# EarthyScience/EasyHybrid.jl

Measured on AMD Instinct MI355X. Metric: training samples/sec, higher is better.
Workload: dtype f32; 1 GPU; RbQ10 hybrid, MLP [2,16,16,1] tanh -> rb (sigmoid-scaled), Q10 global, MSE + Adam(0.01), batch=65536 per GPU, fp32 (BASELINE.json configs[1]); global_batch=65536, resident_batches_per_gpu=64, parallelism=dp1, ranks_seen=1, launcher=none, gradient_exchange=none (one GPU)

## Files before the change

### easyhybrid.jl_amd/csrc/eh_api.hip

```cpp
#include <hip/hip_runtime.h>
#include <chrono>

#include <algorithm>
#include <cfloat>
#include <atomic>
#include <cmath>
#include <cstdarg>
#include <cstdio>
#include <cstdlib>
#include <cstring>
#include <memory>
#include <mutex>
#include <string>
#include <thread>
#include <vector>

#include "eh_internal.hpp"
#include "eh_kernels.hpp"
#include "eh_chain.hpp"
#include "eh_lbfgs.hpp"
#include "eh_wide.hpp"
#include "eh_lform.hpp"
#include "eh_seq.hpp"

// ... 277 lines not shown
    const EhNet& net = h->net;
    EhStepArgs v = *a;
    v.fz.gacc = nullptr;
    v.count = std::min<long long>(a->count, 8192);
    v.bn_update = 0; v.stamps = nullptr; v.slab = h->slab; v.n_acc = h->n_acc;
    v.yhat = nullptr; v.pout = nullptr;
    if (v.count <= 0) return true;
    const int grid = grid_for(h, v.count);
    const size_t nb = (size_t)h->n_acc * sizeof(float);
    float* dev = nullptr;
    if (hipMalloc(&dev, 2 * nb) != hipSuccess) { (void)hipGetLastError(); return true; }
    std::vector<float> host(2 * (size_t)h->n_acc);
    float* sc = h->sc;
    bool launched = true;
    for (int k = 0; k < 2 && launched; ++k) {
        hipError_t e = k == 0 ? h->arch->var[h->variant].launch(EH_MODE_TRAIN, h->act, KFAST(h), grid, h->stream, &net, &v)
                              : eh_jit_launch(&je->k, EH_MODE_TRAIN, grid, h->stream, &net, &v);
        if (e != hipSuccess) { (void)hipGetLastError(); launched = false; break; }
        hipLaunchKernelGGL((eh_reduce_kernel<false, 16>), dim3((h->n_acc + 15) / 16), dim3(256), 0, h->stream, h->slab, grid, h->n_acc, net.n_theta, net.T, 0,
                           dev + (size_t)k * h->n_acc, TH(h), MM(h), VV(h), sc, sc, h->opt, (float*)nullptr, h->img, net.loss, (const float*)nullptr, (const float*)nullptr, 0u);
        if (hipGetLastError() != hipSuccess) { launched = false; break; }
    }
    bool ok = true;
    std::string why;
    if (launched && hipMemcpyAsync(host.data(), dev, 2 * nb, hipMemcpyDeviceToHost, h->stream) == hipSuccess && hipStreamSynchronize(h->stream) == hipSuccess) {
        const float* A = host.data(); const float* B = A + h->n_acc;
        if (getenv("EH_DEBUG_JIT_SKEW")) host[(size_t)h->n_acc + net.n_theta] *= 1.01f;
        double gmax = 0.0, dmax = 0.0;
        for (int i = 0; i < net.n_theta; ++i) { gmax = std::max(gmax, (double)fabsf(A[i])); dmax = std::max(dmax, (double)fabsf(A[i] - B[i])); }
        const double sa = A[net.n_theta], sb = B[net.n_theta];
        bool counts = true;
        for (int t = 0; t < net.T; ++t) counts = counts && A[net.n_theta + 1 + t] == B[net.n_theta + 1 + t];
        const bool loss_ok = (std::isnan(sa) && std::isnan(sb)) || fabs(sa - sb) <= 1e-5 * fabs(sa) + 1e-30;
        if (!(dmax <= 1e-5 * gmax + 1e-30) || !loss_ok || !counts || !std::isfinite(gmax)) {
            ok = false;
            char b[320];
            snprintf(b, sizeof b, "the kernel compiled at run time disagrees with the one built ahead of time on %lld samples of this model's data "
                     "(gradient: max |difference| %.3g against a largest entry of %.3g; loss sum %.9g vs %.9g; valid counts %s): the handle keeps the kernels built ahead of time",
                     v.count, dmax, gmax, sb, sa, counts ? "equal" : "DIFFERENT");
            why = b;
        }
    } else (void)hipGetLastError();
    (void)hipFree(dev);
    if (!ok) { je->state.store(-1); h->jit_failed = true; h->jit_log = why; }
    return ok;
}

static void eh_agg_factors(eh_handle* h) {
    int tdata = 0;
    for (int t = 0; t < h->net.T; ++t) tdata += ((h->roles >> (2 * t)) & 3u) == 0u ? 1 : 0;
    h->img.agg_a = h->agg ? 1.0f / ((float)std::max(1, tdata) * (float)(1 + h->n_extra)) : 1.0f;
    h->img.l2s = h->agg ? 1.0f / (float)(1 + h->n_extra) : 1.0f;
}

static const EhSpecKernel* spec_lookup(const eh_handle* h) {
    static const EhSpecKernel* const list[] = {
#define EH_SPEC_ITEM(k) eh_spec_##k(),
        EH_SPEC_LIST(EH_SPEC_ITEM)
#undef EH_SPEC_ITEM
    };
    static std::mutex mu;
    static uint64_t prepared[sizeof list / sizeof list[0]] = {};
    if (!h->aot_spec || h->lform || h->act == EH_ACT_PER_NET || h->drop_on) return nullptr;
    const EhArchInfo* A = h->arch;
    const EhVariant& V = A->var[h->variant];
    const int kf = KFAST(h);
    for (size_t i = 0; i < sizeof list / sizeof list[0]; ++i) {
        const EhSpecKernel* k = list[i];
        if (k->wide != (A->wide != 0) || k->bf16 != V.bf16 || k->nbi != A->nbi || k->nbh != A->nbh || k->nl != A->nl || k->nt != V.nt || k->nw != V.nw ||
            k->act != h->act || k->fast != kf || (k->so != 0) != (V.so != 0) || memcmp(&k->net, &h->net, sizeof(EhNet)) != 0) continue;
        {
            std::lock_guard<std::mutex> lk(mu);
            const uint64_t bit = 1ull << (h->device & 63);
            if (!(prepared[i] & bit)) {
                if (hipSetDevice(h->device) != hipSuccess || k->prepare() != hipSuccess) { (void)hipGetLastError(); return nullptr; }
                prepared[i] |= bit;
            }
        }
        return k;
    }
    return nullptr;
}

static hipError_t step_launch(eh_handle* h, int mode, int grid, const EhStepArgs* a) {
    if (mode == EH_MODE_TRAIN_ORD) {
        if (const EhSpecKernel* sk = spec_lookup(h)) {
            const hipError_t e = sk->launch(mode, grid, h->stream, &h->net, a);
            if (e == hipSuccess) h->spec_used = sk; else (void)hipGetLastError();
            return e;
        }
        if (jit_wanted(h, EH_MODE_TRAIN)) {
            eh_handle_s::JitEntry* je = jit_entry(h);
            if (je) return (je->verified && je->k.fn[EH_MODE_TRAIN_ORD]) ? eh_jit_launch(&je->k, mode, grid, h->stream, &h->net, a) : hipErrorNotSupported;
        }
        return h->arch->var[h->variant].launch(mode, h->act, KFAST(h), grid, h->stream, &h->net, a);
    }
    if (mode == EH_MODE_TRAIN_MULTI) {
        if (const EhSpecKernel* sk = spec_lookup(h)) {
            if (sk->launch(mode, grid, h->stream, &h->net, a) == hipSuccess) { h->spec_used = sk; return hipSuccess; }
            (void)hipGetLastError();
        } else if (jit_wanted(h, EH_MODE_TRAIN)) {
            eh_handle_s::JitEntry* je = jit_entry(h);
            if (je && je->verified && je->k.fn[EH_MODE_TRAIN_MULTI]) {
                if (eh_jit_launch(&je->k, mode, grid, h->stream, &h->net, a) == hipSuccess) return hipSuccess;
                (void)hipGetLastError();
            }
        }
        return h->arch->var[h->variant].launch(mode, h->act, KFAST(h), grid, h->stream, &h->net, a);
    }
    if (const EhSpecKernel* sk = spec_lookup(h)) {
        const hipError_t e = sk->launch(mode, grid, h->stream, &h->net, a);
        if (e == hipSuccess) { h->spec_used = sk; return e; }
        (void)hipGetLastError();
    }
    if (jit_wanted(h, mode)) {
        eh_handle_s::JitEntry* je = jit_entry(h);
        if (je && !je->verified && mode != EH_MODE_EVAL && !h->capturing && je->spec && h->net.mech != EH_MECH_PROGRAM && h->net.loss != EH_LOSS_PROGRAM &&
            h->act != EH_ACT_PER_NET && !h->drop_on && !getenv("EH_JIT_NO_VERIFY")) {
            bool has_lprog = false;
            for (int t = 0; t < h->net.T; ++t) has_lprog = has_lprog || ((h->net.loss_t >> (4 * t)) & 15u) == (unsigned)EH_LOSS_PROGRAM;
            if (has_lprog || jit_verify(h, je, a)) je->verified = true; else je = nullptr;
        }
        if (je) {
            const hipError_t e = eh_jit_launch(&je->k, mode, grid, h->stream, &h->net, a);
            if (e == hipSuccess) return e;
            (void)hipGetLastError();
            je->state.store(-1); h->jit_failed = true;
            h->jit_log = std::string("launch of the run-time compiled kernel failed: ") + hipGetErrorString(e);
        }
        if ((h->net.loss == EH_LOSS_PROGRAM || h->drop_on) && mode != EH_MODE_EVAL) return hipErrorNotSupported;
    }
    if (h->act == EH_ACT_PER_NET) return hipErrorNotSupported;
    return h->arch->var[h->variant].launch(mode, h->act, KFAST(h), grid, h->stream, &h->net, a);
}

extern "C" {

int32_t eh_version(void) { return EH_ABI_VERSION; }

const char* eh_last_error(const eh_handle* h) { return h ? h->err.c_str() : g_create_err.c_str(); }

static std::mutex g_stage_mu;
static float* g_stage[2] = {nullptr, nullptr};
static size_t g_stage_bytes = 0;
static int copy_out(eh_handle* h, float* dst, const float* src_dev, size_t n);
static void lbfgs_release(eh_handle* h);
static int copy_in(eh_handle* h, float* dst_dev, const float* src, size_t n);
static std::mutex g_stream_pool_mu;
static std::vector<std::pair<int, hipStream_t>> g_stream_pool;
static hipStream_t stream_pool_take(int device) {
    std::lock_guard<std::mutex> lk(g_stream_pool_mu);
    for (size_t i = 0; i < g_stream_pool.size(); ++i)
        if (g_stream_pool[i].first == device) { hipStream_t s = g_stream_pool[i].second; g_stream_pool.erase(g_stream_pool.begin() + (long)i); return s; }
    return nullptr;
}
static void stream_pool_give(int device, hipStream_t s) {
    {
        std::lock_guard<std::mutex> lk(g_stream_pool_mu);
        int kept = 0;
        for (auto& e : g_stream_pool) kept += e.first == device;
        if (kept < 8 && !getenv("EH_NO_STREAM_POOL")) { g_stream_pool.emplace_back(device, s); return; }
    }
    (void)hipStreamDestroy(s);
}

static int seq_desc_check(const eh_model_desc* d) {
    if (d->activation != EH_ACT_PER_NET) return 0;
    const int na = std::min(d->n_nets > 0 ? d->n_nets : d->n_hidden, (int)EH_MAX_NETS);
    int n_lstm = 0, at = -1;
    for (int l = 0; l < na; ++l)
        if (d->net_activation[l] == EH_LAYER_LSTM) { if (at < 0) at = l; ++n_lstm; }
    if (!n_lstm) return 0;
    if (d->n_nets > 0) return fail(nullptr, EH_EUNSUPPORTED, "eh_create: no kernel for a MultiNN sequence model (EH_LAYER_LSTM with n_nets = %d)", d->n_nets);
    if (at == 0) return fail(nullptr, EH_EINVAL, "eh_create: EH_LAYER_LSTM at hidden layer 0: the LSTM layer takes the Dense layer in front of it");
    if (n_lstm > 1) return fail(nullptr, EH_EINVAL, "eh_create: %d EH_LAYER_LSTM layers (one, at hidden layer 1: stacked Recurrence layers are not built)", n_lstm);
    if (d->n_hidden != 3 || at != 1 || d->hidden[2] != d->hidden[1])
        return fail(nullptr, EH_EUNSUPPORTED, "eh_create: no kernel for an LSTM layer at hidden layer %d of %d (built: n_hidden = 3, hidden = [I, H, H], the LSTM at layer 1)", at, d->n_hidden);
    if (d->hidden[0] < 1 || d->hidden[1] < 1) return fail(nullptr, EH_EINVAL, "eh_create: hidden = [%d, %d, ..]", d->hidden[0], d->hidden[1]);
    if (d->hidden[0] > 32 || d->hidden[1] > 32) return fail(nullptr, EH_EUNSUPPORTED, "eh_create: no kernel for LSTM widths I = %d, H = %d (built: up to 32 each)", d->hidden[0], d->hidden[1]);
    if (d->n_predictors > 32) return fail(nullptr, EH_EUNSUPPORTED, "eh_create: no kernel for a sequence model with P = %d predictors (built: up to 32)", d->n_predictors);
    if (d->input_batchnorm) return fail(nullptr, EH_EUNSUPPORTED, "eh_create: no kernel for input BatchNorm on a sequence model (3-D input)");
    if (d->n_targets > 1) return fail(nullptr, EH_EUNSUPPORTED, "eh_create: no kernel for a sequence model with %d targets (built: one)", d->n_targets);
    return 1;
}

int32_t eh_create(const eh_model_desc* d, eh_handle** out) {
    if (!d || !out) return fail(nullptr, EH_EINVAL, "eh_create: null argument");
    *out = nullptr;
    if (d->struct_size != (int32_t)sizeof(eh_model_desc)) return fail(nullptr, EH_EINVAL, "eh_create: struct_size %d != %zu", d->struct_size, sizeof(eh_model_desc));
    MechInfo mi;
    if (!mech_info(d->mech, &mi, d)) return fail(nullptr, EH_EUNSUPPORTED, "eh_create: unknown mechanistic model id %d (no silent fallback)", d->mech);
    const int seqk = (d->activation == EH_ACT_PER_NET && d->n_hidden >= 0 && d->n_hidden <= EH_MAX_HIDDEN && d->n_nets >= 0 && d->n_nets <= EH_MAX_NETS) ? seq_desc_check(d) : 0;
    if (seqk < 0) return seqk;
    const bool seq = seqk == 1;
    if (d->mech == EH_MECH_PROGRAM) {
        if (d->n_params < 1 || d->n_params > EH_MAX_PARAMS) return fail(nullptr, EH_EINVAL, "eh_create: a program takes 1..%d parameters, descriptor has %d", EH_MAX_PARAMS, d->n_params);
        if (d->prog_len < 1 || d->prog_len > EH_MAX_PROG) return fail(nullptr, EH_EUNSUPPORTED, "eh_create: program of %d instructions (1..%d)", d->prog_len, EH_MAX_PROG);
        if (d->prog_n_const < 0 || d->prog_n_const > EH_MAX_PROG_CONST) return fail(nullptr, EH_EUNSUPPORTED, "eh_create: program with %d constants (0..%d)", d->prog_n_const, EH_MAX_PROG_CONST);
        if (d->prog_n_forc < 0 || d->prog_n_forc > EH_MAX_FORC) return fail(nullptr, EH_EINVAL, "eh_create: program with %d forcings (0..%d)", d->prog_n_forc, EH_MAX_FORC);
        if (d->prog_n_out < 1 || d->prog_n_out > EH_MAX_PROG_OUT) return fail(nullptr, EH_EUNSUPPORTED, "eh_create: program with %d outputs (1..%d)", d->prog_n_out, EH_MAX_PROG_OUT);
        auto slot_ok = [&](unsigned sl, int upto) {
            if (sl < EH_PROG_SLOT_FORC) return (int)sl < d->n_params;
            if (sl < EH_PROG_SLOT_CONST) return (int)sl - EH_PROG_SLOT_FORC < d->prog_n_forc;
            if (sl < EH_PROG_SLOT_INSTR) return (int)sl - EH_PROG_SLOT_CONST < d->prog_n_const;
            return (int)sl - EH_PROG_SLOT_INSTR < upto;
        };
        for (int i = 0; i < d->prog_len; ++i) {
            const unsigned w = d->prog_code[i], op = w & 255u;
            if (op >= EH_OP_COUNT) return fail(nullptr, EH_EUNSUPPORTED, "eh_create: program instruction %d has unknown opcode %u", i, op);
            const int nop = (op == EH_OP_SELECT) ? 3 : (op == EH_OP_NEG || op == EH_OP_EXP || op == EH_OP_LOG || op == EH_OP_SQRT || op == EH_OP_TANH ||
                                                        op == EH_OP_SIGMOID || op == EH_OP_ABS || op == EH_OP_SIN || op == EH_OP_COS) ? 1 : 2;
            const unsigned sl[3] = {(w >> 8) & 255u, (w >> 16) & 255u, w >> 24};
            for (int k = 0; k < 3; ++k) {
                if (k < nop ? !slot_ok(sl[k], i) : sl[k] != 0u)
                    return fail(nullptr, EH_EINVAL, "eh_create: program instruction %d, operand %d names slot %u (undefined at that point, or a non-zero unused operand)", i, k, sl[k]);
// ... 276 lines not shown
    }
    tick("pset / bn / gacc");
    h->slab_rows = lform ? (int)EH_LFORM_ROWS : h->max_blocks;
    HIPCHK_C(hipMalloc(&h->slab, (std::max((size_t)h->slab_rows * std::max(h->n_acc, EH_EVAL_STATS * n.T), (size_t)1 << 20) + 16) * sizeof(float)));
    HIPCHK_C(hipMalloc(&h->gradbuf, (size_t)h->n_acc * sizeof(float)));
    HIPCHK_C(hipMalloc(&h->mombuf, EH_MAX_TARG * EH_EVAL_STATS * sizeof(float)));
    HIPCHK_C(hipMemset(h->mombuf, 0, EH_MAX_TARG * EH_EVAL_STATS * sizeof(float)));
    HIPCHK_C(hipMalloc(&h->tcount, 3 * EH_MAX_TARG * sizeof(float)));
    HIPCHK_C(hipMemset(h->tcount, 0, 3 * EH_MAX_TARG * sizeof(float)));
    HIPCHK_C(hipMalloc(&h->inv_n, EH_TT * EH_MAX_TARG * sizeof(float)));
    HIPCHK_C(hipMemset(h->inv_n, 0, EH_TT * EH_MAX_TARG * sizeof(float)));
    HIPCHK_C(hipMemset(h->gradbuf, 0, (size_t)h->n_acc * sizeof(float)));
    tick("slab + small buffers");
    if (seq) {
        std::vector<unsigned char> wf((size_t)n.n_theta, 0);
        const int* o = h->seq_off;
        std::fill(wf.begin() + o[EH_SEQ_WIN], wf.begin() + o[EH_SEQ_BIN], (unsigned char)1);
        std::fill(wf.begin() + o[EH_SEQ_WHD], wf.begin() + o[EH_SEQ_BHD], (unsigned char)1);
        std::fill(wf.begin() + o[EH_SEQ_WOUT], wf.begin() + o[EH_SEQ_BOUT], (unsigned char)1);
        HIPCHK_C(hipMalloc(&h->wflag, wf.size()));
        HIPCHK_C(hipMemcpy(h->wflag, wf.data(), wf.size(), hipMemcpyHostToDevice));
    }
    else if (!lform) { if (int rc = build_maps(h, true)) { g_create_err = h->err; eh_destroy(h); return rc; } }
    else {
        std::vector<unsigned char> wf((size_t)n.n_theta, 0);
        for (int k = 0; k < h->l_nnets; ++k)
            for (int l = 0; l < h->l_net[k].nl; ++l) std::fill(wf.begin() + h->l_net[k].woff[l], wf.begin() + h->l_net[k].boff[l], (unsigned char)1);
        HIPCHK_C(hipMalloc(&h->wflag, wf.size()));
        HIPCHK_C(hipMemcpy(h->wflag, wf.data(), wf.size(), hipMemcpyHostToDevice));
    }
    tick("maps");
    {
        std::vector<float> img0((size_t)arch->img_floats, 0.0f);
        for (int j = 0; j < d->n_params; ++j) {
            if (d->param_kind[j] == EH_PAR_FIXED) img0[arch->phi_off + EH_IMG_PHI + j] = d->param_default[j];
            img0[arch->phi_off + EH_IMG_LO + j] = d->param_lower[j];
            img0[arch->phi_off + EH_IMG_SC + j] = d->param_upper[j] - d->param_lower[j];
        }
        for (int p = 0; p < 32; ++p) { img0[arch->phi_off + EH_IMG_BNM + p] = 0.0f; img0[arch->phi_off + EH_IMG_BNR + p] = d->input_batchnorm ? 1.0f / std::sqrt(1.0f + EH_BN_EPS) : 1.0f; }
        for (int k = 0; k < (lform ? 0 : n_nets); ++k)
            for (int l = net_d[k]; l < nl; ++l)
                for (int i = 0; i < net_w[k][l]; ++i)
                    img0[arch->wh_off + (size_t)(l - 1) * arch->hp * arch->sh + (size_t)(h->net_r0[k][l] + i) * arch->sh + h->net_r0[k][l - 1] + i] = 1.0f;
        auto put_int = [&](int slot, int v) { memcpy(&img0[arch->phi_off + slot], &v, sizeof(int)); };
        if (!lform && !seq) {
            for (int l = 0; l <= d->n_hidden; ++l) { put_int(EH_IMG_WOFF + l, lw_off[l]); put_int(EH_IMG_BOFF + l, lb_off[l]); }
            for (int l = 0; l < d->n_hidden; ++l) put_int(EH_IMG_WIDTH + l, tot_w[l]);
        }
        for (int j = 0; j < d->n_params; ++j)
            if (d->param_kind[j] == EH_PAR_GLOBAL) put_int(EH_IMG_GPAR + d->param_index[j], j);
        HIPCHK_C(hipMalloc(&h->image, img0.size() * sizeof(float)));
        HIPCHK_C(hipMemcpy(h->image, img0.data(), img0.size() * sizeof(float), hipMemcpyHostToDevice));
        EhImg& im = h->img;
        im.image = h->image; im.imap = h->imap; im.g_off = n.g_off; im.phi_off = arch->phi_off;
        im.l2c = 0.0f; im.l2w = nullptr; im.n_theta = n.n_theta; im.b_off = arch->b_off; im.wflag = h->wflag;
        im.agg_a = 1.0f; im.l2s = 1.0f;
        HIPCHK_C(hipMalloc(&h->l2val, sizeof(float)));
        HIPCHK_C(hipMemset(h->l2val, 0, sizeof(float)));
        {
            int nw = 0;
            if (seq) nw = (h->seq_off[EH_SEQ_BIN] - h->seq_off[EH_SEQ_WIN]) + (h->seq_off[EH_SEQ_BHD] - h->seq_off[EH_SEQ_WHD]) + (h->seq_off[EH_SEQ_BOUT] - h->seq_off[EH_SEQ_WOUT]);
            else if (lform) { for (int k = 0; k < h->l_nnets; ++k) for (int l = 0; l < h->l_net[k].nl; ++l) nw += h->l_net[k].in[l] * h->l_net[k].out[l]; }
            else for (const EhEntry& e : enumerate_entries(h)) nw += e.col >= 0 ? 1 : 0;
            h->n_weights = nw;
        }
        for (int j = 0; j < d->n_params; ++j)
            if (d->param_kind[j] == EH_PAR_GLOBAL) {
                const int g = d->param_index[j];
                im.glob_par[g] = j; im.glo[g] = d->param_lower[j]; im.ghi[g] = d->param_upper[j];
            }
        tick("image");
        hipLaunchKernelGGL(eh_image_kernel, dim3((unsigned)((nt + 255) / 256)), dim3(256), 0, h->stream, TH(h), (int)nt, h->img);
        HIPCHK_C(hipGetLastError());
        tick("image kernel launch");
        HIPCHK_C(hipStreamSynchronize(h->stream));
        tick("synchronize");
    }
#undef HIPCHK_C
    if (h->act == EH_ACT_PER_NET && !h->lform && !h->seq && !jit_entry(h)) {
        const std::string log = h->jit_log;
        eh_destroy(h);
        return fail(nullptr, EH_EUNSUPPORTED, "eh_create: per-net activations need the run-time compiled kernel, which failed to build: %.600s", log.c_str());
    }
    *out = h;
    return EH_OK;
}

int32_t eh_destroy(eh_handle* h) {
    if (!h) return EH_OK;
    (void)hipSetDevice(h->device);
    if (h->own_stream) (void)hipStreamSynchronize(h->own_stream);
    for (auto e : h->ev) (void)hipEventDestroy(e);
    for (auto& g : h->graphs) (void)hipGraphExecDestroy(g.exec);
    for (auto& e : h->jit) { if (e->worker.joinable()) e->worker.join(); eh_jit_release(&e->k); }
    eh_comm_release(h);
    (void)hipSetDevice(h->device);
    (void)hipFree(h->pset); (void)hipFree(h->opt_tab);
    (void)hipFree(h->gacc); (void)hipFree(h->ord); if (h->ord_err) (void)hipHostFree(h->ord_err); (void)hipFree(h->bn_part); (void)hipFree(h->bn_run); (void)hipFree(h->bn_shift); (void)hipFree(h->bn_stat); (void)hipFree(h->tcount); (void)hipFree(h->mombuf); (void)hipFree(h->slab); (void)hipFree(h->gradbuf); (void)hipFree(h->inv_n);
    (void)hipFree(h->prog); (void)hipFree(h->l2val); (void)hipFree(h->l2w); (void)hipFree(h->loss_hist); (void)hipFree(h->perm); (void)hipFree(h->out_buf); (void)hipFree(h->idx_buf);
    eval_host_release(h);
    lbfgs_release(h);
    (void)hipFree(h->mech_ws); (void)hipFree(h->l_ws); (void)hipFree(h->l_split); (void)hipFree(h->l_dk); (void)hipFree(h->l_lprog); (void)hipFree(h->wflag);
    (void)hipFree(h->stamps); (void)hipFree(h->image); (void)hipFree(h->imap); (void)hipFree(h->rmap);
    (void)hipFree(h->split[0].recs); (void)hipFree(h->split[1].recs); (void)hipFree(h->split[0].starts); (void)hipFree(h->split[1].starts); (void)hipFree(h->seq_ws); (void)hipFree(h->chain_part);
    if (h->own_stream) stream_pool_give(h->device, h->own_stream);
    delete h;
    return EH_OK;
}

int32_t eh_n_theta(const eh_handle* h, int64_t* n) {
    if (!h || !n) return EH_EINVAL;
    *n = h->net.n_theta;
    return EH_OK;
}

int32_t eh_set_stream(eh_handle* h, void* s) {
    if (!h) return EH_EINVAL;
    h->stream = s ? (hipStream_t)s : h->own_stream;
    return EH_OK;
}

int32_t eh_synchronize(eh_handle* h) {
    if (!h) return EH_EINVAL;
    HIPCHK(h, hipSetDevice(h->device));
    FLUSH(h);
    HIPCHK(h, hipStreamSynchronize(h->stream));
    if (h->p2p_on) {
        unsigned c[3] = {0, 0, 0};
        HIPCHK(h, hipMemcpy(c, h->p2p_ctr, sizeof c, hipMemcpyDeviceToHost));
        if (c[1]) return fail(h, EH_EHIP, "eh_synchronize: a cross-GPU exchange ran into its 2 s deadline (a rank is missing or out of step); results are invalid");
    }
    if (h->ord_err && *(volatile unsigned*)h->ord_err)
        return fail(h, EH_EHIP, "eh_synchronize: an ordered step's row of sums did not arrive within its 2 s deadline; results are invalid");
    return EH_OK;
}

static int set_loss_program(eh_handle* h, int target, const uint32_t* code, int32_t n_instr, const float* consts, int32_t n_const, int32_t out_slot, const char* who) {
    if (!h || !code || (n_const > 0 && !consts)) return EH_EINVAL;
    if (h->seq) return fail(h, EH_EUNSUPPORTED, "%s: recorded losses are not built for sequence models", who);
    if (n_instr < 1 || n_instr > EH_MAX_PROG) return fail(h, EH_EUNSUPPORTED, "%s: %d instructions (1..%d)", who, n_instr, EH_MAX_PROG);
    if (n_const < 0 || n_const > EH_MAX_PROG_CONST) return fail(h, EH_EUNSUPPORTED, "%s: %d constants (0..%d)", who, n_const, EH_MAX_PROG_CONST);
    auto slot_ok = [&](unsigned sl, int upto) {
        if (sl < EH_PROG_SLOT_CONST) return sl < 2u;
        if (sl < EH_PROG_SLOT_INSTR) return (int)sl - EH_PROG_SLOT_CONST < n_const;
        return (int)sl - EH_PROG_SLOT_INSTR < upto;
    };
    for (int i = 0; i < n_instr; ++i) {
        const unsigned w = code[i], op = w & 255u;
        if (op >= EH_OP_COUNT) return fail(h, EH_EUNSUPPORTED, "%s: instruction %d has unknown opcode %u", who, i, op);
        const int nop = (op == EH_OP_SELECT) ? 3 : (op == EH_OP_NEG || op == EH_OP_EXP || op == EH_OP_LOG || op == EH_OP_SQRT || op == EH_OP_TANH ||
                                                    op == EH_OP_SIGMOID || op == EH_OP_ABS || op == EH_OP_SIN || op == EH_OP_COS) ? 1 : 2;
        const unsigned sl[3] = {(w >> 8) & 255u, (w >> 16) & 255u, w >> 24};
        for (int k = 0; k < 3; ++k)
            if (k < nop ? !slot_ok(sl[k], i) : sl[k] != 0u) return fail(h, EH_EINVAL, "%s: instruction %d, operand %d names slot %u (undefined at that point, or a non-zero unused operand)", who, i, k, sl[k]);
    }
    if (out_slot < 0 || !slot_ok((unsigned)out_slot, n_instr)) return fail(h, EH_EINVAL, "%s: output slot %d", who, out_slot);
    if (h->net.loss == EH_LOSS_PROGRAM) { HIPCHK(h, hipSetDevice(h->device)); FLUSH(h); }
    EhLossProg1& lp = target < 0 ? static_cast<EhLossProg1&>(h->loss_prog) : h->loss_prog.per[target];
    lp.code.assign(code, code + n_instr);
    lp.consts.assign(consts, consts + n_const);
    lp.out = out_slot;
    h->loss_prog.gen++;
    return EH_OK;
}
int32_t eh_set_loss_program(eh_handle* h, const uint32_t* code, int32_t n_instr, const float* consts, int32_t n_const, int32_t out_slot) {
    if (h) for (int t = 0; t < EH_MAX_TARG; ++t) h->loss_prog.per[t] = EhLossProg1();
    return set_loss_program(h, -1, code, n_instr, consts, n_const, out_slot, "eh_set_loss_program");
}
int32_t eh_set_target_loss_program(eh_handle* h, int32_t target, const uint32_t* code, int32_t n_instr, const float* consts, int32_t n_const, int32_t out_slot) {
    if (!h) return EH_EINVAL;
    if (target < 0 || target >= h->net.T) return fail(h, EH_EINVAL, "eh_set_target_loss_program: target %d of %d", target, h->net.T);
    return set_loss_program(h, target, code, n_instr, consts, n_const, out_slot, "eh_set_target_loss_program");
}

int32_t eh_set_target_losses(eh_handle* h, const int32_t* kinds, int32_t n) {
    if (!h || !kinds) return EH_EINVAL;
    if (n != h->net.T) return fail(h, EH_EINVAL, "eh_set_target_losses: %d losses for %d targets", n, h->net.T);
    unsigned lt = 0;
    bool same = true;
    bool any_prog = false, any_two = false;
    for (int t = 0; t < n; ++t) {
        if (kinds[t] < EH_LOSS_MSE || kinds[t] > EH_LOSS_PROGRAM) return fail(h, EH_EUNSUPPORTED, "eh_set_target_losses: loss %d for target %d is not implemented on the device", kinds[t], t);
        lt |= (unsigned)kinds[t] << (4 * t);
        same = same && kinds[t] == kinds[0];
        any_prog = any_prog || kinds[t] == EH_LOSS_PROGRAM;
        if (kinds[t] == EH_LOSS_PROGRAM && !h->loss_prog.has(t)) return fail(h, EH_ESTATE, "eh_set_target_losses: target %d: EH_LOSS_PROGRAM without a program (eh_set_loss_program / eh_set_target_loss_program first)", t);
        any_two = any_two || (kinds[t] >= EH_LOSS_PEARSONLOSS && kinds[t] <= EH_LOSS_PBKGELOSS) || (kinds[t] == EH_LOSS_RMSE && n > 1);
    }
    if (same) return eh_set_option(h, "training_loss", kinds[0]);
    if (any_two && h->fused) return fail(h, EH_EUNSUPPORTED, "rmse (on a multi-target model) / pearson / kge training losses take forward passes ahead of the step: switch fused_update off first");
    HIPCHK(h, hipSetDevice(h->device));
    FLUSH(h);
    h->net.loss = any_prog ? EH_LOSS_PROGRAM : EH_LOSS_MSE;
    h->net.loss_t = lt;
    {
        const int want = h->lform ? 0 : fast_wanted(h->arch, h->net.K, h->net.P, h->net.T, h->net.mech);
        const int fast = any_two ? 0 : (want & h->fast_user);
        if (!h->lform && fast != h->fast) { h->fast = fast; return build_maps(h, false); }
    }
    return EH_OK;
}

int32_t eh_set_target_roles(eh_handle* h, const int32_t* roles, int32_t n) {
    if (!h || !roles) return EH_EINVAL;
    if (n != h->net.T) return fail(h, EH_EINVAL, "eh_set_target_roles: %d roles for %d targets", n, h->net.T);
    unsigned r = 0;
    int ndata = 0;
    for (int t = 0; t < n; ++t) {
        if (roles[t] < 0 || roles[t] > 2) return fail(h, EH_EINVAL, "eh_set_target_roles: role %d of target %d (0 data, 1 extra-loss mean, 2 extra-loss sum)", roles[t], t);
        r |= (unsigned)roles[t] << (2 * t);
        ndata += roles[t] == 0;
    }
    if (ndata == 0) return fail(h, EH_EINVAL, "eh_set_target_roles: at least one data target");
    if (r != 0 && h->net.T < 2) return fail(h, EH_EINVAL, "eh_set_target_roles: an extra-loss entry is a target of its own");
    HIPCHK(h, hipSetDevice(h->device));
    FLUSH(h);
    h->roles = r;
    eh_agg_factors(h);
    return EH_OK;
}

int32_t eh_jit_status(eh_handle* h, int32_t* n_compiled, char* log, int64_t log_bytes) {
    if (!h || !n_compiled) return EH_EINVAL;
    int n = 0;
    for (auto& e : h->jit) n += e->state.load(std::memory_order_acquire) > 0 ? 1 : 0;
    std::string msg = h->jit_log;
    if (h->spec_used && h->aot_spec) { n += 1; msg = std::string("ahead-of-time: ") + h->spec_used->what + (msg.empty() ? "" : "; ") + msg; }
    *n_compiled = n;
    if (log && log_bytes > 0) {
        const size_t m = std::min((size_t)log_bytes - 1, msg.size());
        memcpy(log, msg.data(), m);
        log[m] = 0;
    }
    return EH_OK;
}

static bool so_allowed(const eh_handle* h) {
    static const bool no_so = getenv("EH_NO_DIRECT_STORE") != nullptr || getenv("EH_NO_SAMPLE_OWNED") != nullptr;
    return !no_so && h->n_nets == 1 && h->desc.n_nets == 0;
}

int32_t eh_set_option(eh_handle* h, const char* name, int64_t value) {
    if (!h || !name) return EH_EINVAL;
    if (h->seq) {
        if (!strcmp(name, "fused_update")) {
            if (value < 0 || value > 2) return fail(h, EH_EINVAL, "fused_update must be 0, 1 or 2");
            if (value == 1) return fail(h, EH_EUNSUPPORTED, "fused_update: the one-kernel step is not built for sequence models (they run the step + reduce pair)");
            return EH_OK;
        }
        if (!strcmp(name, "multi_step") || !strcmp(name, "specialize") || !strcmp(name, "precision")) {
            if (value) return fail(h, EH_EUNSUPPORTED, "%s: not built for sequence models (one fp32 kernel family, one launch per step)", name);
            return EH_OK;
        }
        if (!strcmp(name, "fast_paths") || !strcmp(name, "row_split") || !strcmp(name, "variant") || !strcmp(name, "aot_spec") || !strcmp(name, "bn_in_kernel")) return EH_OK;
        if (!strcmp(name, "jit")) { h->jit_on = value != 0; return EH_OK; }
        if (!strcmp(name, "training_loss")) {
            if (value < EH_LOSS_MSE || value > EH_LOSS_PROGRAM) return fail(h, EH_EUNSUPPORTED, "training_loss %lld is not implemented on the device", (long long)value);
            if (value > EH_LOSS_NSELOSS) return fail(h, EH_EUNSUPPORTED, "training_loss %lld: sequence models train on mse, rmse, mae and nseLoss (the two-pass losses and recorded losses are not built for them)", (long long)value);
            h->net.loss = (int)value;
            h->net.loss_t = (unsigned)value;
            return EH_OK;
        }
    }
    if (h->lform && (!strcmp(name, "fast_paths") || !strcmp(name, "row_split") || !strcmp(name, "variant") || !strcmp(name, "precision"))) {
        if (!strcmp(name, "precision") && value) return fail(h, EH_EUNSUPPORTED, "precision: the layer-wise form computes in fp32");
        return EH_OK;
    }
    if (h->drop_on && value && (!strcmp(name, "precision") || !strcmp(name, "row_split")))
        return fail(h, EH_EUNSUPPORTED, "%s: dropout is built for the fp32 per-wave kernels only (eh_set_dropout with all rates zero removes it)", name);
    if (!strcmp(name, "lbfgs_one_max")) {
        if (value < -1 || value > INT32_MAX) return fail(h, EH_EINVAL, "lbfgs_one_max must be -1 or a parameter count");
        h->lb_one_max = (int)value;
        return EH_OK;
    }
    if (!strcmp(name, "max_blocks")) {
        if (value < 1 || value > 256) return fail(h, EH_EINVAL, "max_blocks must be 1..256 (one workgroup per CU)");
        h->max_blocks = (int)value;
        return EH_OK;
    }
    if (!strcmp(name, "bn_in_kernel")) {
        h->bn_no_self = value == 0;
        return EH_OK;
    }
    if (!strcmp(name, "multi_step")) {
        h->multi_step = value != 0;
        return EH_OK;
    }
    if (!strcmp(name, "eval_blocks")) {
        if (value < 0 || value > 4096) return fail(h, EH_EINVAL, "eval_blocks must be 0 (default) .. 4096");
        h->eval_blocks = (int)value;
        return EH_OK;
    }
    if (!strcmp(name, "mech_blocks")) {
        if (value < 0 || value > EH_MECH_MAXROWS) return fail(h, EH_EINVAL, "mech_blocks must be 0 (no cap) .. %d", (int)EH_MECH_MAXROWS);
        h->mech_blocks = (int)value;
        return EH_OK;
    }
    if (!strcmp(name, "mech_tiles")) {
        if (value < 1 || value > 1024) return fail(h, EH_EINVAL, "mech_tiles must be 1..1024");
        h->mech_tiles = (int)value;
        return EH_OK;
    }
    if (!strcmp(name, "fast_paths")) {
        const int want = fast_wanted(h->arch, h->net.K, h->net.P, h->net.T, h->net.mech);
        h->fast_user = value ? (int)value : 0;
        h->fast = (h->net.loss >= EH_LOSS_PEARSONLOSS) ? 0 : (want & h->fast_user);
        HIPCHK(h, hipSetDevice(h->device));
        FLUSH(h);
        return build_maps(h, false);
    }
    if (!strcmp(name, "fused_update")) {
        if (value && two_pass_mask(h->net)) return fail(h, EH_EUNSUPPORTED, "fused_update: rmse (on a multi-target model) / pearson / kge training losses take forward passes ahead of the step");
        if (value && (h->img.l2c != 0.0f || h->img.l2w)) return fail(h, EH_EUNSUPPORTED, "fused_update: the weight_l2 extra loss is not built for it");
        if (value && h->arch->wide) return fail(h, EH_EUNSUPPORTED, "fused_update is not built for hidden widths above 64");
        if (!value && h->p2p_alloc) return fail(h, EH_ESTATE, "fused_update: eh_p2p_disable first");
        if (value < 0 || value > 2) return fail(h, EH_EINVAL, "fused_update must be 0, 1 or 2");
        if (value == 1 && h->chain.n) return fail(h, EH_EUNSUPPORTED, "fused_update: the one-kernel step is not built for an optimiser chain (ClipNorm needs the norm of the whole gradient before any element moves): 0 or 2 run the step + reduce + chain kernels");
        HIPCHK(h, hipSetDevice(h->device));
        FLUSH(h);
        h->fused = value != 0;
        h->fused_det = value == 2;
        return EH_OK;
    }
    if (!strcmp(name, "training_loss")) {
        if (value < EH_LOSS_MSE || value > EH_LOSS_PROGRAM) return fail(h, EH_EUNSUPPORTED, "training_loss %lld is not implemented on the device", (long long)value);
        if (value == EH_LOSS_PROGRAM)
            for (int t = 0; t < h->net.T; ++t)
                if (!h->loss_prog.has(t)) return fail(h, EH_ESTATE, "training_loss EH_LOSS_PROGRAM: call eh_set_loss_program first");
        const bool two = (value >= EH_LOSS_PEARSONLOSS && value <= EH_LOSS_PBKGELOSS) || (value == EH_LOSS_RMSE && h->net.T > 1);
        if (two && h->fused) return fail(h, EH_EUNSUPPORTED, "rmse (on a multi-target model) / pearson / kge training losses take forward passes ahead of the step: switch fused_update off first");
        HIPCHK(h, hipSetDevice(h->device));
        FLUSH(h);
        h->net.loss = (int)value;
        h->net.loss_t = 0;
        for (int t = 0; t < h->net.T; ++t) h->net.loss_t |= (unsigned)value << (4 * t);
        if (!h->lform) {
            const int want = fast_wanted(h->arch, h->net.K, h->net.P, h->net.T, h->net.mech);
            const int fast = (two || value >= EH_LOSS_PEARSONLOSS) ? 0 : (want & h->fast_user);
            if (fast != h->fast) { h->fast = fast; return build_maps(h, false); }
        }
        return EH_OK;
    }
    if (!strcmp(name, "jit")) {
        h->jit_on = value != 0;
        return EH_OK;
    }
    if (!strcmp(name, "agg") || !strcmp(name, "extra_terms")) {
        if (!strcmp(name, "agg")) { if (value != 0 && value != 1) return fail(h, EH_EINVAL, "agg must be 0 (sum) or 1 (mean)"); }
        else if (value < 0 || value > 64) return fail(h, EH_EINVAL, "extra_terms must be 0..64");
        HIPCHK(h, hipSetDevice(h->device));
        FLUSH(h);
        if (!strcmp(name, "agg")) h->agg = (int)value; else h->n_extra = (int)value;
        eh_agg_factors(h);
        return EH_OK;
    }
    if (!strcmp(name, "check_idx")) {
        h->check_idx = value != 0;
        return EH_OK;
    }
    if (!strcmp(name, "p2p_mode")) {
        if (value != 0 && value != 1) return fail(h, EH_EINVAL, "p2p_mode must be 0 (election in the step's epilogue) or 1 (publish from the next kernel's prologue)");
        if (!h->p2p_on) return fail(h, EH_ESTATE, "p2p_mode: no peer-to-peer exchange on this handle (eh_p2p_init / eh_p2p_init_local first)");
        HIPCHK(h, hipSetDevice(h->device));
        FLUSH(h);
        HIPCHK(h, hipStreamSynchronize(h->stream));
        h->p2p_host.mode = (int)value;
        HIPCHK(h, hipMemcpy(h->p2p_dev, &h->p2p_host, sizeof(EhP2P), hipMemcpyHostToDevice));
        return EH_OK;
    }
    if (!strcmp(name, "empty_target_nan")) {
        h->empty_nan = value != 0;
        return EH_OK;
    }
    if (!strcmp(name, "aot_spec")) {
        h->aot_spec = value != 0;
        return EH_OK;
    }
    if (!strcmp(name, "specialize")) {
        h->specialize = value != 0;
        h->specialize_async = value == 2;
        return EH_OK;
    }
    if (!strcmp(name, "row_split")) {
        const bool now = h->arch->wide != 0;
        if ((value != 0) == now) return EH_OK;
        if (!h->arch_alt) return fail(h, EH_EUNSUPPORTED, "row_split: this model has only the %s kernel", now ? "row-split" : "per-wave");
        if (value && h->fused) return fail(h, EH_EUNSUPPORTED, "row_split: switch fused_update off first");
        if (h->arch->var[h->variant].bf16) return fail(h, EH_ESTATE, "row_split: the bf16-forward kernels exist in the row-split family only (set precision 0 first)");
        HIPCHK(h, hipSetDevice(h->device));
        FLUSH(h);
        std::swap(h->arch, h->arch_alt);
        h->variant = (h->arch->nvar > 1 && !h->arch->wide) ? 1 : 0;
        h->fast = (h->net.loss >= EH_LOSS_PEARSONLOSS) ? 0 : (fast_wanted(h->arch, h->net.K, h->net.P, h->net.T, h->net.mech) & h->fast_user);
        for (int vi = 0; vi < h->arch->nvar; ++vi) HIPCHK(h, h->arch->var[vi].prepare());
        return build_maps(h, false);
    }
    if (!strcmp(name, "precision")) {
        if (value < 0 || value > 2) return fail(h, EH_EINVAL, "precision must be 0 (f32), 1 (bf16 forward / fp32-exact backward) or 2 (bf16 operands in both passes, fp32 accumulate)");
        const int now = h->arch->var[h->variant].bf16;
        if ((int)value == now) return EH_OK;
        if (value) {
            if (h->act == EH_ACT_SWISH || h->act == EH_ACT_PER_NET)
                return fail(h, EH_EUNSUPPORTED, "precision: the bf16 kernels keep only the rounded activation (tanh / sigmoid / relu / identity; not swish, not per-net activations)");
            if (h->fused) return fail(h, EH_EUNSUPPORTED, "precision: switch fused_update off first (the row-split kernels have no such mode)");
            const EhArchInfo* W = h->arch->wide ? h->arch : h->arch_alt;
            const bool so_ok = so_allowed(h);
            int vb = -1;
            if (W && so_ok) for (int vi = 0; vi < W->nvar; ++vi) if (W->var[vi].bf16 == (int)value && W->var[vi].so) { vb = vi; break; }
            if (W && vb < 0) for (int vi = 0; vi < W->nvar; ++vi) if (W->var[vi].bf16 == (int)value && !W->var[vi].so) { vb = vi; break; }
            if (vb < 0) return fail(h, EH_EUNSUPPORTED, "precision: no bf16 kernel is built for this shape (row-split shapes only: hidden width 33..128)");
            HIPCHK(h, hipSetDevice(h->device));
            FLUSH(h);
            if (W != h->arch) { std::swap(h->arch, h->arch_alt); h->fast = 0; }
            h->variant = vb;
            for (int vi = 0; vi < h->arch->nvar; ++vi) HIPCHK(h, h->arch->var[vi].prepare());
        } else {
            HIPCHK(h, hipSetDevice(h->device));
            FLUSH(h);
            h->variant = 0;
        }
        return build_maps(h, false);
    }
    if (!strcmp(name, "variant")) {
        if (value < 0 || value >= h->arch->nvar) return fail(h, EH_EINVAL, "variant must be 0..%d for this shape", h->arch->nvar - 1);
        if (h->arch->var[value].bf16 != h->arch->var[h->variant].bf16) return fail(h, EH_EINVAL, "variant %lld belongs to the other precision (set the \"precision\" option)", (long long)value);
        if (h->arch->var[value].so && !so_allowed(h))
            return fail(h, EH_EUNSUPPORTED, "variant %lld is the sample-owned training kernel: one-network models only (and not with EH_NO_DIRECT_STORE / EH_NO_SAMPLE_OWNED set)", (long long)value);
        h->variant = (int)value;
        HIPCHK(h, hipSetDevice(h->device));
        return build_maps(h, false);
    }
    return fail(h, EH_EINVAL, "unknown option %s", name);
}

int32_t eh_set_data(eh_handle* h, int32_t split, int64_t n, const float* x, const float* const* forcings, const float* const* targets,
                    int32_t on_device) {
    if (!h) return EH_EINVAL;
    if (split != EH_SPLIT_TRAIN && split != EH_SPLIT_VAL) return fail(h, EH_EINVAL, "eh_set_data: split %d", split);
    if (n < 0 || n > 0x7fffffffLL) return fail(h, EH_EINVAL, "eh_set_data: n = %lld", (long long)n);
    if (on_device & ~(EH_DATA_ON_DEVICE | EH_DATA_X_PLANES | EH_DATA_X_ROWS)) return fail(h, EH_EINVAL, "eh_set_data: flags %d", on_device);
    if ((on_device & EH_DATA_X_ROWS) && (on_device & (EH_DATA_ON_DEVICE | EH_DATA_X_PLANES))) return fail(h, EH_EINVAL, "eh_set_data: EH_DATA_X_ROWS goes with host arrays only, and not with EH_DATA_X_PLANES");
    if (n > 0 && ((!x && h->net.P > 0) || !forcings || !targets)) return fail(h, EH_EINVAL, "eh_set_data: null array");
    const EhNet& net = h->net;
    HIPCHK(h, hipSetDevice(h->device));
    EhSplit& sp = h->split[split];
    HIPCHK(h, hipStreamSynchronize(h->stream));
    (void)hipFree(sp.recs); (void)hipFree(sp.starts);
    sp.recs = nullptr; sp.n = 0; sp.starts = nullptr; sp.nwin = 0;
    if (split == EH_SPLIT_TRAIN) h->perm_valid = false;
    if (n == 0) return EH_OK;
    const int C = h->C;
    static const bool dbg_t = getenv("EH_DEBUG_SET_DATA") != nullptr;
    const auto t_a = std::chrono::steady_clock::now();
    HIPCHK(h, hipMalloc(&sp.recs, (size_t)n * C * sizeof(float)));
// ... 1411 lines not shown
    if (!h) return EH_EINVAL;
    if (split != EH_SPLIT_TRAIN && split != EH_SPLIT_VAL) return fail(h, EH_EINVAL, "eh_loss_and_grad: split %d", split);
    HIPCHK(h, hipSetDevice(h->device));
    FLUSH(h);
    EhSplit& sp = h->split[split];
    int rc;
    const int* didx = nullptr;
    if (idx) {
        if ((rc = stage_host_idx(h, sp, idx, 0, count, "eh_loss_and_grad"))) return rc;
        didx = h->idx_buf;
        first = 0;
    } else {
        rc = check_window(h, sp, first, count, "eh_loss_and_grad");
        if (rc) return rc;
    }
    rc = do_step(h, sp, didx, first, count, false, false, nullptr);
    if (rc) return rc;
    std::vector<float> host((size_t)h->n_acc);
    HIPCHK(h, hipMemcpyAsync(host.data(), h->gradbuf, host.size() * sizeof(float), hipMemcpyDeviceToHost, h->stream));
    HIPCHK(h, hipStreamSynchronize(h->stream));
    const int nt = h->net.n_theta;
    if (grad) memcpy(grad, host.data(), (size_t)nt * sizeof(float));
    if (loss) {
        *loss = host[nt];
        if (h->empty_nan && h->net.T > 1) {
            bool some = false, empty = false;
            for (int t = 0; t < h->net.T; ++t) { some = some || host[nt + 1 + t] > 0.0f; empty = empty || !(host[nt + 1 + t] > 0.0f); }
            if (some && empty) *loss = std::nanf("");
        }
    }
    if (n_valid) {
        double c = 0;
        for (int t = 0; t < h->net.T; ++t) c += host[nt + 1 + t];
        *n_valid = (int64_t)std::llround(c);
    }
    return EH_OK;
}

int32_t eh_get_bn_state(eh_handle* h, float* running_mean, float* running_var, int64_t n) {
    if (!h || !running_mean || !running_var) return EH_EINVAL;
    if (!h->bn_on) return fail(h, EH_ESTATE, "eh_get_bn_state: the model has no input BatchNorm");
    if (n != h->net.P) return fail(h, EH_EINVAL, "eh_get_bn_state: n = %lld, model has %d predictors", (long long)n, h->net.P);
    HIPCHK(h, hipSetDevice(h->device));
    FLUSH(h);
    HIPCHK(h, hipStreamSynchronize(h->stream));
    HIPCHK(h, hipMemcpy(running_mean, h->bn_run, (size_t)n * sizeof(float), hipMemcpyDeviceToHost));
    HIPCHK(h, hipMemcpy(running_var, h->bn_run + 32, (size_t)n * sizeof(float), hipMemcpyDeviceToHost));
    return EH_OK;
}

int32_t eh_set_bn_state(eh_handle* h, const float* running_mean, const float* running_var, int64_t n) {
    if (!h || !running_mean || !running_var) return EH_EINVAL;
    if (!h->bn_on) return fail(h, EH_ESTATE, "eh_set_bn_state: the model has no input BatchNorm");
    if (n != h->net.P) return fail(h, EH_EINVAL, "eh_set_bn_state: n = %lld, model has %d predictors", (long long)n, h->net.P);
    HIPCHK(h, hipSetDevice(h->device));
    FLUSH(h);
    HIPCHK(h, hipStreamSynchronize(h->stream));
    std::vector<float> rstd((size_t)n);
    for (int64_t p = 0; p < n; ++p) rstd[p] = 1.0f / std::sqrt(running_var[p] + EH_BN_EPS);
    HIPCHK(h, hipMemcpy(h->bn_run, running_mean, (size_t)n * sizeof(float), hipMemcpyHostToDevice));
    HIPCHK(h, hipMemcpy(h->bn_run + 32, running_var, (size_t)n * sizeof(float), hipMemcpyHostToDevice));
    HIPCHK(h, hipMemcpy(h->image + h->arch->phi_off + EH_IMG_BNM, running_mean, (size_t)n * sizeof(float), hipMemcpyHostToDevice));
    HIPCHK(h, hipMemcpy(h->image + h->arch->phi_off + EH_IMG_BNR, rstd.data(), (size_t)n * sizeof(float), hipMemcpyHostToDevice));
    return EH_OK;
}

int32_t eh_opt_init(eh_handle* h, int32_t rule, float lr, float beta1, float beta2, float eps, float weight_decay) {
    if (!h) return EH_EINVAL;
    if (rule < EH_OPT_ADAM || rule > EH_OPT_DESCENT) return fail(h, EH_EUNSUPPORTED, "eh_opt_init: unknown rule %d", rule);
    HIPCHK(h, hipSetDevice(h->device));
    FLUSH(h);
    HIPCHK(h, hipStreamSynchronize(h->stream));
    if (h->lb) h->lb->active = false;
    h->opt = EhOpt{rule, lr, beta1, beta2, eps, weight_decay, nullptr};
    h->opt_groups = 1;
    h->chain = EhChain{}; h->chain_gen = 0;
    const size_t nt = (size_t)h->net.n_theta;
    HIPCHK(h, hipMemset(MM(h), 0, nt * sizeof(float)));
    HIPCHK(h, hipMemset(VV(h), 0, nt * sizeof(float)));
    const float sc[4] = {beta1, beta2, beta1, beta2};
    HIPCHK(h, hipMemcpy(h->sc, sc, sizeof sc, hipMemcpyHostToDevice));
    h->sc_sel = 0;
    h->opt_ready = true;
    return EH_OK;
}

int32_t eh_opt_init_groups(eh_handle* h, const uint8_t* group, int64_t n_theta, int32_t n_groups, const int32_t* rule, const float* hyper) {
    if (!h) return EH_EINVAL;
    if (!group || !rule || !hyper) return fail(h, EH_EINVAL, "eh_opt_init_groups: null table");
    if (n_theta != h->net.n_theta) return fail(h, EH_EINVAL, "eh_opt_init_groups: n_theta %lld, the model has %d", (long long)n_theta, h->net.n_theta);
    if (n_groups > EH_MAX_OPT_GROUPS) return fail(h, EH_EUNSUPPORTED, "eh_opt_init_groups: %d groups (at most %d)", n_groups, EH_MAX_OPT_GROUPS);
    if (n_groups < 1) return fail(h, EH_EINVAL, "eh_opt_init_groups: %d groups", n_groups);
    for (int k = 0; k < n_groups; ++k)
        if (rule[k] < EH_OPT_ADAM || rule[k] > EH_OPT_DESCENT) return fail(h, EH_EUNSUPPORTED, "eh_opt_init_groups: group %d: unknown rule %d", k, rule[k]);
    const size_t nt = (size_t)n_theta;
    for (size_t i = 0; i < nt; ++i)
        if (group[i] >= n_groups) return fail(h, EH_EINVAL, "eh_opt_init_groups: element %zu in group %d of %d", i, (int)group[i], n_groups);
    HIPCHK(h, hipSetDevice(h->device));
    FLUSH(h);
    HIPCHK(h, hipStreamSynchronize(h->stream));
    const size_t tab_bytes = offsetof(EhOptTab, gid) + ((nt + 3) & ~(size_t)3);
    std::vector<unsigned char> host(tab_bytes, 0);
    EhOptTab* const t = reinterpret_cast<EhOptTab*>(host.data());
    for (int k = 0; k < n_groups; ++k) {
        const float* hp = hyper + 5 * k;
        t->r[k] = EhOpt{rule[k], hp[0], hp[1], hp[2], hp[3], hp[4], nullptr};
    }
    t->n = n_groups;
    memcpy(host.data() + offsetof(EhOptTab, gid), group, nt);
    if (!h->opt_tab) HIPCHK(h, hipMalloc(&h->opt_tab, tab_bytes));
    HIPCHK(h, hipMemcpy(h->opt_tab, host.data(), tab_bytes, hipMemcpyHostToDevice));
    h->opt = EhOpt{EH_OPT_ADAM, t->r[0].lr, t->r[0].b1, t->r[0].b2, t->r[0].eps, t->r[0].wd, h->opt_tab};
    h->opt_groups = n_groups;
    if (h->lb) h->lb->active = false;
    h->chain = EhChain{}; h->chain_gen = 0;
    HIPCHK(h, hipMemset(MM(h), 0, nt * sizeof(float)));
    HIPCHK(h, hipMemset(VV(h), 0, nt * sizeof(float)));
    float sc[4 * EH_MAX_OPT_GROUPS] = {};
    for (int k = 0; k < n_groups; ++k) {
        sc[4 * k] = sc[4 * k + 2] = hyper[5 * k + 1];
        sc[4 * k + 1] = sc[4 * k + 3] = hyper[5 * k + 2];
    }
    HIPCHK(h, hipMemcpy(h->sc, sc, sizeof sc, hipMemcpyHostToDevice));
    h->sc_sel = 0;
    h->opt_ready = true;
    return EH_OK;
}

int32_t eh_opt_init_chain(eh_handle* h, const eh_opt_stage* stages, int32_t n_stages, int32_t rule, float lr, float beta1, float beta2, float eps, float weight_decay) {
    if (!h || !stages) return EH_EINVAL;
    if (n_stages < 1) return fail(h, EH_EINVAL, "eh_opt_init_chain: %d stages", n_stages);
    if (n_stages > EH_MAX_OPT_STAGES) return fail(h, EH_EUNSUPPORTED, "eh_opt_init_chain: %d stages (at most %d, nested chains flattened)", n_stages, EH_MAX_OPT_STAGES);
    if (rule < EH_OPT_ADAM || rule > EH_OPT_DESCENT) return fail(h, EH_EUNSUPPORTED, "eh_opt_init_chain: unknown rule %d", rule);
    EhChain c{};
    c.n = n_stages; c.i_norm = -1; c.i_rule = -1; c.p = 2;
    for (int k = 0; k < n_stages; ++k) {
        const eh_opt_stage& st = stages[k];
        c.kind[k] = st.kind; c.a[k] = st.a;
        if (st.kind == EH_STAGE_RULE) {
            if (c.i_rule >= 0) return fail(h, EH_EUNSUPPORTED, "eh_opt_init_chain: stage %d: a second rule (a chain holds exactly one of Adam / AdamW / RMSProp / Descent)", k);
            c.i_rule = k;
        } else if (st.kind == EH_STAGE_CLIPGRAD) {
            if (!(st.a >= 0.0f)) return fail(h, EH_EINVAL, "eh_opt_init_chain: stage %d: ClipGrad(delta = %g)", k, (double)st.a);
        } else if (st.kind == EH_STAGE_WEIGHTDECAY) {
            if (!(st.a >= 0.0f)) return fail(h, EH_EINVAL, "eh_opt_init_chain: stage %d: WeightDecay(lambda = %g)", k, (double)st.a);
        } else if (st.kind == EH_STAGE_CLIPNORM) {
            if (!(st.a > 0.0f)) return fail(h, EH_EINVAL, "eh_opt_init_chain: stage %d: ClipNorm(omega = %g)", k, (double)st.a);
            if (c.i_norm >= 0) return fail(h, EH_EUNSUPPORTED, "eh_opt_init_chain: stage %d: a second ClipNorm (one norm pass per step is built)", k);
            if (c.i_rule >= 0) return fail(h, EH_EUNSUPPORTED, "eh_opt_init_chain: stage %d: ClipNorm behind the rule needs the norm of the UPDATE, a second pass over it: not built", k);
            if (st.b == 1.0f) c.p = 1; else if (st.b == 2.0f) c.p = 2; else if (st.b == INFINITY) c.p = 0;
            else return fail(h, EH_EUNSUPPORTED, "eh_opt_init_chain: stage %d: ClipNorm with p = %g (1, 2 and Inf are built)", k, (double)st.b);
            c.i_norm = k; c.omega = st.a; c.thr = st.flags & 1;
        } else return fail(h, EH_EUNSUPPORTED, "eh_opt_init_chain: stage %d: unknown kind %d", k, st.kind);
    }
    if (c.i_rule < 0) return fail(h, EH_EUNSUPPORTED, "eh_opt_init_chain: no EH_STAGE_RULE among the stages (a chain holds exactly one rule)");
    if (h->fused && !h->fused_det) return fail(h, EH_EUNSUPPORTED, "eh_opt_init_chain: the one-kernel step (fused_update 1) is not built for an optimiser chain: switch it to 0 or 2 first");
    if (h->p2p_alloc) return fail(h, EH_EUNSUPPORTED, "eh_opt_init_chain: the peer-to-peer fused exchange is not built for an optimiser chain: eh_p2p_disable first");
    int rc = eh_opt_init(h, rule, lr, beta1, beta2, eps, weight_decay);
    if (rc) return rc;
    if (!h->chain_part) HIPCHK(h, hipMalloc(&h->chain_part, (EH_CHAIN_PARTS + 3) * sizeof(double)));
    HIPCHK(h, hipMemset(h->chain_part, 0, (EH_CHAIN_PARTS + 3) * sizeof(double)));
    static int gen = 0;
    h->chain = c; h->chain_gen = ++gen;
    return EH_OK;
}

int32_t eh_opt_chain_status(eh_handle* h, int64_t* n_applied, int64_t* n_clipped, int64_t* n_nonfinite) {
    if (!h) return EH_EINVAL;
    if (!h->chain.n) return fail(h, EH_ESTATE, "eh_opt_chain_status: no optimiser chain (call eh_opt_init_chain first)");
    HIPCHK(h, hipSetDevice(h->device));
    FLUSH(h);
    HIPCHK(h, hipStreamSynchronize(h->stream));
    unsigned long long ctr[3];
    HIPCHK(h, hipMemcpy(ctr, h->chain_part + EH_CHAIN_PARTS, sizeof ctr, hipMemcpyDeviceToHost));
    if (n_applied) *n_applied = (int64_t)ctr[0];
    if (n_clipped) *n_clipped = (int64_t)ctr[1];
    if (n_nonfinite) *n_nonfinite = (int64_t)ctr[2];
    return EH_OK;
}

static void lbfgs_release(eh_handle* h) {
    if (!h->lb) return;
    (void)hipFree(h->lb->vec); (void)hipFree(h->lb->dbl); (void)hipFree(h->lb->trace); (void)hipFree(h->lb->idx);
    delete h->lb;
    h->lb = nullptr;
}

static int lbfgs_ready(eh_handle* h, const char* who) {
    if (!h->lb || !h->lb->active) return fail(h, EH_ESTATE, "%s: call eh_lbfgs_init first (eh_opt_init* leaves L-BFGS mode)", who);
    if (h->capturing) return fail(h, EH_EUNSUPPORTED, "%s: graph capture is not built for L-BFGS", who);
    return EH_OK;
}

int32_t eh_lbfgs_init(eh_handle* h, const eh_lbfgs_opts* o) {
    if (!h || !o) return EH_EINVAL;
    if (o->m < 1 || o->m > EH_LBFGS_MAX_M) return fail(h, EH_EINVAL, "eh_lbfgs_init: m = %d (1..%d)", o->m, (int)EH_LBFGS_MAX_M);
    if (!(o->c1 > 0.0 && o->c1 < o->c2 && o->c2 < 1.0)) return fail(h, EH_EINVAL, "eh_lbfgs_init: need 0 < c1 < c2 < 1 (c1 = %g, c2 = %g)", o->c1, o->c2);
    if (o->max_linesearch < 1 || o->max_linesearch > 48) return fail(h, EH_EINVAL, "eh_lbfgs_init: max_linesearch = %d (1..48)", o->max_linesearch);
    if (!(o->g_tol >= 0.0) || !(o->f_reltol >= 0.0)) return fail(h, EH_EINVAL, "eh_lbfgs_init: g_tol = %g, f_reltol = %g (both >= 0)", o->g_tol, o->f_reltol);
    if (!(o->initial_step >= 0.0) || !std::isfinite(o->initial_step)) return fail(h, EH_EINVAL, "eh_lbfgs_init: initial_step = %g (>= 0; 0 = min(1, 1 / ||g||))", o->initial_step);
    if (h->capturing) return fail(h, EH_EUNSUPPORTED, "eh_lbfgs_init: graph capture is not built for L-BFGS");
    if (h->drop_on) return fail(h, EH_EUNSUPPORTED, "eh_lbfgs_init: dropout: the line search needs the same objective at every trial point, the masks change with every pass (eh_set_dropout with all rates zero removes it)");
    if (h->bn_on) return fail(h, EH_EUNSUPPORTED, "eh_lbfgs_init: input BatchNorm: the reference's Optimization.jl driver never carries the layer state, and that path is not built");
    if (h->comm || h->lgroup || h->p2p_on || h->p2p_alloc) return fail(h, EH_EUNSUPPORTED, "eh_lbfgs_init: data parallelism (a communicator or a peer-to-peer group on this handle) is not built for L-BFGS");
    HIPCHK(h, hipSetDevice(h->device));
    FLUSH(h);
    HIPCHK(h, hipStreamSynchronize(h->stream));
    const size_t n = (size_t)h->net.n_theta;
// ... 134 lines not shown
                             double* record, double* trace_row, int32_t* wrote_row) {
    if (!o || !state || !gram || !sums || !record || !trace_row) return EH_EINVAL;
    if (o->m < 1 || o->m > EH_LBFGS_MAX_M || o->max_linesearch < 1 || o->max_linesearch > 48) return EH_EINVAL;
    const int w = eh_lb_decide(*o, maxiters, state, gram, sums, f, n_valid, record, trace_row);
    if (wrote_row) *wrote_row = w;
    return EH_OK;
}

int32_t eh_get_opt_beta_t(eh_handle* h, float* bt, int32_t n_groups) {
    if (!h || !bt) return EH_EINVAL;
    if (n_groups != h->opt_groups) return fail(h, EH_EINVAL, "eh_get_opt_beta_t: %d groups, the handle has %d", n_groups, h->opt_groups);
    HIPCHK(h, hipSetDevice(h->device));
    FLUSH(h);
    HIPCHK(h, hipStreamSynchronize(h->stream));
    float sc[4 * EH_MAX_OPT_GROUPS];
    HIPCHK(h, hipMemcpy(sc, h->sc, sizeof sc, hipMemcpyDeviceToHost));
    for (int k = 0; k < n_groups; ++k) { bt[2 * k] = sc[4 * k + 2 * h->sc_sel]; bt[2 * k + 1] = sc[4 * k + 2 * h->sc_sel + 1]; }
    return EH_OK;
}

int32_t eh_set_opt_beta_t(eh_handle* h, const float* bt, int32_t n_groups) {
    if (!h || !bt) return EH_EINVAL;
    if (!h->opt_ready) return fail(h, EH_ESTATE, "eh_set_opt_beta_t: call eh_opt_init or eh_opt_init_groups first");
    if (n_groups != h->opt_groups) return fail(h, EH_EINVAL, "eh_set_opt_beta_t: %d groups, the handle has %d", n_groups, h->opt_groups);
    HIPCHK(h, hipSetDevice(h->device));
    FLUSH(h);
    HIPCHK(h, hipStreamSynchronize(h->stream));
    for (int k = 0; k < n_groups; ++k)
        HIPCHK(h, hipMemcpy(h->sc + 4 * k + 2 * h->sc_sel, bt + 2 * k, 2 * sizeof(float), hipMemcpyHostToDevice));
    return EH_OK;
}

int32_t eh_get_opt_state(eh_handle* h, float* m, float* v, int64_t n, float* beta_t) {
    if (!h) return EH_EINVAL;
    if (n != h->net.n_theta) return fail(h, EH_EINVAL, "eh_get_opt_state: n");
    HIPCHK(h, hipSetDevice(h->device));
    FLUSH(h);
    HIPCHK(h, hipStreamSynchronize(h->stream));
    if (m) { if (int rc = copy_out(h, m, MM(h), (size_t)n)) return rc; }
    if (v) { if (int rc = copy_out(h, v, VV(h), (size_t)n)) return rc; }
    if (beta_t) HIPCHK(h, hipMemcpy(beta_t, h->sc + 2 * h->sc_sel, 2 * sizeof(float), hipMemcpyDeviceToHost));
    return EH_OK;
}

int32_t eh_set_opt_state(eh_handle* h, const float* m, const float* v, int64_t n, const float* beta_t) {
    if (!h) return EH_EINVAL;
    if (!h->opt_ready) return fail(h, EH_ESTATE, "eh_set_opt_state: call eh_opt_init first");
    if (n != h->net.n_theta) return fail(h, EH_EINVAL, "eh_set_opt_state: n");
    HIPCHK(h, hipSetDevice(h->device));
    FLUSH(h);
    HIPCHK(h, hipStreamSynchronize(h->stream));
    if (m) { if (int rc = copy_in(h, MM(h), m, (size_t)n)) return rc; }
    if (v) { if (int rc = copy_in(h, VV(h), v, (size_t)n)) return rc; }
    if (beta_t) HIPCHK(h, hipMemcpy(h->sc + 2 * h->sc_sel, beta_t, 2 * sizeof(float), hipMemcpyHostToDevice));
    return EH_OK;
}

int32_t eh_set_dropout(eh_handle* h, const float* rate, int32_t n_hidden, uint64_t seed, uint64_t step) {
    if (!h) return EH_EINVAL;
    if (!rate || n_hidden != h->desc.n_hidden) return fail(h, EH_EINVAL, "eh_set_dropout: %d rates for %d hidden layers", (int)n_hidden, (int)h->desc.n_hidden);
    bool any = false;
    for (int l = 0; l < n_hidden; ++l) {
        if (!(rate[l] >= 0.0f && rate[l] < 1.0f)) return fail(h, EH_EINVAL, "eh_set_dropout: rate[%d] = %g (0 <= p < 1)", l, (double)rate[l]);
        any = any || rate[l] > 0.0f;
    }
    if (any) {
        const char* why = nullptr;
        if (h->seq) why = "sequence models";
        else if (h->lform) why = "the layer-wise form (more than 3 hidden layers or widths above 128)";
        else if (h->desc.n_nets != 0) why = "MultiNN models";
        else if (h->arch->var[h->variant].bf16) why = "the bf16 kernels (precision option)";
        else if (h->arch->wide) why = "the row-split kernels (hidden widths above 64, or the row_split option)";
        else if (h->p2p_on || h->p2p_alloc || h->comm || h->lgroup) why = "data parallelism (a communicator or a peer-to-peer exchange is set up on this handle)";
        else if (h->capturing) why = "a handle that is recording a graph";
        if (why) return fail(h, EH_EUNSUPPORTED, "eh_set_dropout: dropout is built for the fp32 per-wave fused kernels of single-network models, not for %s", why);
        if (!h->jit_on) return fail(h, EH_EUNSUPPORTED, "eh_set_dropout: the dropout kernels are compiled at run time and the jit option is off (EH_JIT=0)");
    }
    HIPCHK(h, hipSetDevice(h->device));
    FLUSH(h);
    h->drop_on = any;
    for (int l = 0; l < EH_MAX_HIDDEN; ++l) h->drop[l] = (any && l < n_hidden) ? rate[l] : 0.0f;
    h->drop_seed = seed; h->drop_step = step;
    if (any) { h->jit_failed = false; h->jit_log.clear(); }
    return EH_OK;
}

int32_t eh_get_dropout(eh_handle* h, float* rate, int32_t cap, uint64_t* seed, uint64_t* step) {
    if (!h) return EH_EINVAL;
    if (rate) {
        if (cap < h->desc.n_hidden) return fail(h, EH_EINVAL, "eh_get_dropout: room for %d rates, the model has %d hidden layers", (int)cap, (int)h->desc.n_hidden);
        for (int l = 0; l < h->desc.n_hidden; ++l) rate[l] = h->drop[l];
    }
    if (seed) *seed = h->drop_seed;
    if (step) *step = h->drop_step;
    return EH_OK;
}

int32_t eh_dropout_mask(eh_handle* h, int32_t layer, uint64_t step, int64_t count, uint8_t* keep) {
    if (!h || !keep) return EH_EINVAL;
    if (layer < 0 || layer >= h->desc.n_hidden || count < 0 || count > (1LL << 24)) return fail(h, EH_EINVAL, "eh_dropout_mask: layer %d, count %lld", (int)layer, (long long)count);
    if (h->desc.n_nets != 0) return fail(h, EH_EUNSUPPORTED, "eh_dropout_mask: single-network models only");
    const int width = h->desc.hidden[layer];
    if (count == 0) return EH_OK;
    HIPCHK(h, hipSetDevice(h->device));
    const size_t n = (size_t)count * (size_t)width;
    uint8_t* dev = nullptr;
    HIPCHK(h, hipMalloc(&dev, n));
    const int nq = (width + 3) / 4;
    const long long work = (long long)count * nq;
    hipLaunchKernelGGL(eh_dropout_mask_kernel, dim3((unsigned)((work + 255) / 256)), dim3(256), 0, h->stream, (unsigned long long)h->drop_seed, (unsigned long long)step, (int)layer, width,
                       (long long)count, eh_drop_threshold(h->drop[layer]), dev);
    hipError_t e = hipGetLastError();
    if (e == hipSuccess) e = hipMemcpyAsync(keep, dev, n, hipMemcpyDeviceToHost, h->stream);
    if (e == hipSuccess) e = hipStreamSynchronize(h->stream);
    (void)hipFree(dev);
    HIPCHK(h, e);
    return EH_OK;
}

int32_t eh_train_step(eh_handle* h, const int32_t* idx, int32_t idx_on_device, int64_t first, int64_t count, float* loss_out) {
    if (!h) return EH_EINVAL;
    if (!h->opt_ready) return fail(h, EH_ESTATE, "eh_train_step: call eh_opt_init first");
    HIPCHK(h, hipSetDevice(h->device));
    EhSplit& sp = h->split[EH_SPLIT_TRAIN];
    int rc;
    const int* didx = nullptr;
    if (idx && !idx_on_device) {
        if ((rc = stage_host_idx(h, sp, idx, first, count, "eh_train_step"))) return rc;
        didx = h->idx_buf;
        first = 0;
    } else if (idx) {
        if (!sp.recs || sp.n == 0) return fail(h, EH_ESTATE, "eh_train_step: no data set for this split (call eh_set_data)");
        if (first < 0 || count < 0) return fail(h, EH_EINVAL, "eh_train_step: first %lld, count %lld", (long long)first, (long long)count);
        didx = idx;
        if (h->check_idx && count > 0) {
            if (h->capturing) return fail(h, EH_ESTATE, "eh_train_step: the check_idx option synchronises: not while a graph is recorded");
            unsigned* bad = nullptr;
            HIPCHK(h, hipMalloc(&bad, 2 * sizeof(unsigned)));
            HIPCHK(h, hipMemsetAsync(bad, 0, sizeof(unsigned), h->stream));
            HIPCHK(h, hipMemsetAsync(bad + 1, 0xFF, sizeof(unsigned), h->stream));
            hipLaunchKernelGGL(eh_idx_check_kernel, dim3((unsigned)std::min<long long>(1024, (count + 255) / 256)), dim3(256), 0, h->stream, idx, (long long)first, (long long)count, (long long)sp.samples(), bad);
            unsigned res[2] = {0, 0};
            hipError_t e = hipGetLastError();
            if (e == hipSuccess) e = hipMemcpyAsync(res, bad, sizeof res, hipMemcpyDeviceToHost, h->stream);
            if (e == hipSuccess) e = hipStreamSynchronize(h->stream);
            (void)hipFree(bad);
            HIPCHK(h, e);
            if (res[0]) return fail(h, EH_EINVAL, "eh_train_step: %u of the %lld device-side indices are outside 0..%lld (first offender: idx[%lld])", res[0], (long long)count, (long long)sp.samples() - 1, (long long)first + (long long)res[1]);
        }
    } else if ((rc = check_window(h, sp, first, count, "eh_train_step"))) return rc;
    rc = ensure_loss_hist(h, 1);
    if (rc) return rc;
    const int grid = h->seq ? 0 : grid_for(h, count);
    bool done = false;
    if (h->fused && !(h->fused_det && grid != 1) && !h->chain.n) {
        rc = do_fused_step(h, sp, didx, first, count, loss_out ? h->loss_hist : nullptr);
        if (rc) return rc;
        done = true;
    } else if (ord_ok(h, grid)) {
        rc = do_fused_step(h, sp, didx, first, count, loss_out ? h->loss_hist : nullptr, true, &done);
        if (rc) return rc;
    }
    if (done) {
        if (loss_out) FLUSH(h);
    } else {
        FLUSH(h);
// ... 302 lines not shown
    HIPCHK(h, hipSetDevice(h->device));
    HIPCHK(h, hipStreamSynchronize(h->stream));
    HIPCHK(h, hipMemcpy(h->bn_shift, shift, (size_t)n * sizeof(float), hipMemcpyHostToDevice));
    return EH_OK;
}

int32_t eh_dp_bn_stats(eh_handle* h, int64_t first, int64_t count) {
    if (!h) return EH_EINVAL;
    if (h->seq) return fail(h, EH_EUNSUPPORTED, "eh_dp_bn_stats: data parallelism is not built for sequence models");
    if (h->lb && h->lb->active) return fail(h, EH_EUNSUPPORTED, "eh_dp_bn_stats: the handle is in L-BFGS mode, which is not built for data parallelism (eh_opt_init* leaves the mode)");
    if (h->drop_on) return fail(h, EH_EUNSUPPORTED, "eh_dp_bn_stats: dropout is not built for data parallelism (the masks are drawn per handle, from its own step count)");
    if (!h->bn_on) return fail(h, EH_ESTATE, "eh_dp_bn_stats: the model has no input BatchNorm");
    HIPCHK(h, hipSetDevice(h->device));
    EhSplit& sp = h->split[EH_SPLIT_TRAIN];
    int rc = check_window(h, sp, first, count, "eh_dp_bn_stats");
    if (rc) return rc;
    const int* idx = h->perm_valid ? h->perm : nullptr;
    const int nblk = (int)std::max<long long>(1, std::min<long long>(32, (count + 1023) / 1024));
    hipLaunchKernelGGL(eh_bn_stats_kernel, dim3(nblk), dim3(1024), 0, h->stream, sp.recs, h->C, h->net.P, idx, (int)first, (int)count, h->bn_part, h->bn_shift);
    HIPCHK(h, hipGetLastError());
    hipLaunchKernelGGL(eh_bn_fold_kernel, dim3(1), dim3(64), 0, h->stream, h->bn_part, nblk, (int)count, h->bn_stat);
    HIPCHK(h, hipGetLastError());
    h->bn_ext = true;
    return EH_OK;
}

int32_t eh_dp_apply(eh_handle* h, float* loss_out) {
    if (!h) return EH_EINVAL;
    if (h->seq) return fail(h, EH_EUNSUPPORTED, "eh_dp_apply: data parallelism is not built for sequence models");
    if (h->lb && h->lb->active) return fail(h, EH_EUNSUPPORTED, "eh_dp_apply: the handle is in L-BFGS mode, which is not built for data parallelism (eh_opt_init* leaves the mode)");
    if (h->drop_on) return fail(h, EH_EUNSUPPORTED, "eh_dp_apply: dropout is not built for data parallelism (the masks are drawn per handle, from its own step count)");
    if (!h->opt_ready) return fail(h, EH_ESTATE, "eh_dp_apply: call eh_opt_init first");
    HIPCHK(h, hipSetDevice(h->device));
    int rc = ensure_loss_hist(h, 1);
    if (rc) return rc;
    float* sc_in = h->sc + 2 * h->sc_sel;
    float* sc_out = h->sc + 2 * (h->sc_sel ^ 1);
    const int nt = h->net.n_theta;
    const bool l2 = h->img.l2c != 0.0f || h->img.l2w;
    if (l2) {
        hipLaunchKernelGGL(eh_weight_l2_kernel, dim3(1), dim3(256), 0, h->stream, TH(h), h->img, h->l2val);
        HIPCHK(h, hipGetLastError());
    }
    if (h->chain.n) {
        if ((rc = launch_chain(h, true, sc_in, sc_out, h->loss_hist))) return rc;
    } else {
        hipLaunchKernelGGL(eh_apply_kernel, dim3((nt + 255) / 256), dim3(256), 0, h->stream, h->gradbuf, nt, TH(h), MM(h), VV(h), sc_in, sc_out, h->opt,
                           h->loss_hist, h->img, h->net.loss, h->net.T, l2 ? h->l2val : nullptr, two_pass_mask(h->net) ? h->inv_n : nullptr, two_pass_mask(h->net));
        HIPCHK(h, hipGetLastError());
    }
    h->sc_sel ^= 1;
    if (loss_out) {
        HIPCHK(h, hipMemcpyAsync(loss_out, h->loss_hist, sizeof(float), hipMemcpyDeviceToHost, h->stream));
        HIPCHK(h, hipStreamSynchronize(h->stream));
    }
    return EH_OK;
}

int32_t eh_device_buffer(eh_handle* h, int32_t which, void** dev_ptr, int64_t* n_floats) {
    if (!h || !dev_ptr || !n_floats) return EH_EINVAL;
    if (h->fused && which != EH_BUF_GRAD && which != EH_BUF_GACC && which != EH_BUF_BNSTAT && which != EH_BUF_TCOUNT && which != EH_BUF_MOMENT) return fail(h, EH_ESTATE, "eh_device_buffer: parameter buffers ping-pong in fused_update mode; switch it off first");
    switch (which) {
        case EH_BUF_GRAD: *dev_ptr = h->gradbuf; *n_floats = h->n_acc; return EH_OK;
        case EH_BUF_THETA: *dev_ptr = TH(h); *n_floats = h->net.n_theta; return EH_OK;
        case EH_BUF_OPT_M: *dev_ptr = MM(h); *n_floats = h->net.n_theta; return EH_OK;
        case EH_BUF_OPT_V: *dev_ptr = VV(h); *n_floats = h->net.n_theta; return EH_OK;
        case EH_BUF_GACC: *dev_ptr = h->gacc; *n_floats = (int64_t)3 * EH_GSHARDS * h->n_acc; return EH_OK;
        case EH_BUF_BNSTAT:
            if (!h->bn_on) return fail(h, EH_ESTATE, "eh_device_buffer: the model has no input BatchNorm");
            *dev_ptr = h->bn_stat; *n_floats = 65; return EH_OK;
        case EH_BUF_TCOUNT: *dev_ptr = h->tcount; *n_floats = 3 * EH_MAX_TARG; return EH_OK;
        case EH_BUF_MOMENT: *dev_ptr = h->mombuf; *n_floats = EH_MAX_TARG * EH_EVAL_STATS; return EH_OK;
        default: return fail(h, EH_EINVAL, "eh_device_buffer: which = %d", which);
    }
}

int32_t eh_debug_stamps(eh_handle* h, uint64_t* out, int32_t n) {
    if (!h || !out || n < 0 || n > EH_STAMP_WORDS) return EH_EINVAL;
    HIPCHK(h, hipSetDevice(h->device));
    if (!h->stamps) {
        HIPCHK(h, hipMalloc(&h->stamps, EH_STAMP_WORDS * sizeof(unsigned long long)));
        HIPCHK(h, hipMemset(h->stamps, 0, EH_STAMP_WORDS * sizeof(unsigned long long)));
        memset(out, 0, (size_t)n * sizeof(uint64_t));
        return EH_OK;
    }
    HIPCHK(h, hipStreamSynchronize(h->stream));
    HIPCHK(h, hipMemcpy(out, h->stamps, (size_t)n * sizeof(uint64_t), hipMemcpyDeviceToHost));
    return EH_OK;
}

int32_t eh_profile_enable(eh_handle* h, int32_t on) {
    if (!h) return EH_EINVAL;
    h->prof = on != 0;
    h->prof_stride = on > 1 ? on : 1;
    h->prof_k = 0;
    h->ev_used = 0;
    return EH_OK;
}

int32_t eh_profile_samples(eh_handle* h, double* ms, int64_t cap, int64_t* n_out) {
    if (!h || !n_out || (cap > 0 && !ms)) return EH_EINVAL;
    HIPCHK(h, hipSetDevice(h->device));
    HIPCHK(h, hipStreamSynchronize(h->stream));
    const int64_t n = std::min<int64_t>((int64_t)(h->ev_used / 3), cap);
    for (int64_t i = 0; i < n; ++i) {
        float t = 0;
        HIPCHK(h, hipEventElapsedTime(&t, h->ev[3 * i], h->ev[3 * i + 2]));
        ms[i] = t;
    }
    *n_out = n;
    return EH_OK;
}

int32_t eh_profile_read(eh_handle* h, int64_t* n_launches, double* mean_ms_step_kernel, double* mean_ms_reduce_kernel) {
    if (!h) return EH_EINVAL;
    HIPCHK(h, hipSetDevice(h->device));
    HIPCHK(h, hipStreamSynchronize(h->stream));
    double a = 0, b = 0;
    const size_t n = h->ev_used / 3;
    for (size_t i = 0; i < n; ++i) {
        float ms = 0;
        HIPCHK(h, hipEventElapsedTime(&ms, h->ev[3 * i], h->ev[3 * i + 1]));
        a += ms;
        HIPCHK(h, hipEventElapsedTime(&ms, h->ev[3 * i + 1], h->ev[3 * i + 2]));
        b += ms;
    }
    if (n_launches) *n_launches = (int64_t)n;
    if (mean_ms_step_kernel) *mean_ms_step_kernel = n ? a / n : 0.0;
    if (mean_ms_reduce_kernel) *mean_ms_reduce_kernel = n ? b / n : 0.0;
    h->ev_used = 0;
    return EH_OK;
}

}
```

### easyhybrid.jl_amd/csrc/eh_arch.hpp

```cpp
#pragma once
#include "eh_device.hpp"

struct EhVariant {
    int nt, nw;
    size_t lds_bytes;
    int red_floats;
    hipError_t (*prepare)(void);
    hipError_t (*launch)(int mode, int act, int fast, int grid, hipStream_t stream, const EhNet* net, const EhStepArgs* args);
    int tiles;
    int bf16;
    int so;
    size_t lds_eval;
};

struct EhArchInfo {
    int nbi, nbh, nl;
    int ip, hp, s0, sh, w0_off, wh_off, wo_off, b_off, phi_off, img_floats;
    int has_fast;
    int nvar;
    EhVariant var[8];
    int wide;
};

struct EhSpecKernel {
    EhNet net;
    int wide, bf16, nbi, nbh, nl, nt, nw, act, fast;
    int so;
    size_t lds_bytes;
    const char* what;
    hipError_t (*prepare)(void);
    hipError_t (*launch)(int mode, int grid, hipStream_t stream, const EhNet* net, const EhStepArgs* args);
};
#define EH_SPEC_LIST(X) X(0) X(1) X(2) X(3) X(4) X(5) X(6)
#define EH_SPEC_DECL(k) extern "C" const EhSpecKernel* eh_spec_##k(void);
EH_SPEC_LIST(EH_SPEC_DECL)
#undef EH_SPEC_DECL

constexpr size_t EH_LDS_LIMIT = 160 * 1024;

template <int NBI, int NBH, int NL>
constexpr int eh_pick_nt() {
    if (sizeof(float) * EhGeom<NBI, NBH, NL, 4, 4>::TOTAL_FLOATS <= EH_LDS_LIMIT) return 4;
    if (sizeof(float) * EhGeom<NBI, NBH, NL, 2, 4>::TOTAL_FLOATS <= EH_LDS_LIMIT) return 2;
    return 1;
}

#define EH_ARCH_LIST(X) \
    X(1, 1, 1) X(1, 1, 2) X(1, 1, 3) \
    X(1, 2, 1) X(1, 2, 2) X(1, 2, 3) \
    X(1, 4, 1) X(1, 4, 2) X(1, 4, 3) \
    X(2, 1, 1) X(2, 1, 2) X(2, 1, 3) \
    X(2, 2, 1) X(2, 2, 2) X(2, 2, 3) \
    X(2, 4, 1) X(2, 4, 2) X(2, 4, 3)

#define EH_WIDE_LIST(X) \
    X(1, 4, 1) X(1, 4, 2) X(1, 4, 3) X(2, 4, 1) X(2, 4, 2) X(2, 4, 3) \
    X(1, 8, 1) X(1, 8, 2) X(2, 8, 1) X(2, 8, 2)

#define EH_ARCH_DECL(a, b, c) extern "C" const EhArchInfo* eh_arch_##a##_##b##_##c(void);
EH_ARCH_LIST(EH_ARCH_DECL)
#undef EH_ARCH_DECL
#define EH_ARCH_DECL(a, b, c) extern "C" const EhArchInfo* eh_wide_##a##_##b##_##c(void);
EH_WIDE_LIST(EH_ARCH_DECL)
#undef EH_ARCH_DECL
```

### easyhybrid.jl_amd/csrc/eh_device.hpp

```cpp
#pragma once
#ifndef __HIPCC_RTC__
#include <hip/hip_runtime.h>
#include <stdint.h>
#endif

#include "easyhybrid_hip.h"

#define EH_BN_SELF_MAX 512
#define EH_EVAL_STATS 8

typedef float f32x4 __attribute__((ext_vector_type(4)));

enum { EH_MODE_TRAIN = 0, EH_MODE_EVAL = 1, EH_MODE_TRAIN_P2P = 2, EH_MODE_TRAIN_MULTI = 3, EH_MODE_TRAIN_ORD = 4 };

struct EhNet {
    int P, K, G, T, F;
    int n_theta, g_off;
    int scale_nn, mech, n_par;
    int loss;
    int n_out;
    unsigned targ_out;
    unsigned par_kind;
    unsigned par_idx;
    unsigned forc_col;
// ... 166 lines not shown
}
__device__ __forceinline__ float eh_ord_group_fold(const float (&g)[EH_ORD_GROUPS]) {
    float t = 0.0f;
#pragma unroll
    for (int k = 0; k < EH_ORD_GROUPS; ++k) t += g[k];
    return t;
}
typedef unsigned u32x4_ord __attribute__((ext_vector_type(4)));
__device__ __forceinline__ __amdgpu_buffer_rsrc_t eh_ord_rsrc(const float* base, int nfloats) {
    return __builtin_amdgcn_make_buffer_rsrc(const_cast<float*>(base), (short)0, 4 * nfloats, 0x00020000);
}
__device__ __forceinline__ f32x4 eh_ord_ld16(__amdgpu_buffer_rsrc_t r, int off) { return __builtin_bit_cast(f32x4, __builtin_amdgcn_raw_buffer_load_b128(r, off, 0, 16)); }
__device__ __forceinline__ void eh_ord_st16(__amdgpu_buffer_rsrc_t r, int off, f32x4 v) { __builtin_amdgcn_raw_buffer_store_b128(__builtin_bit_cast(u32x4_ord, v), r, off, 0, 16); }
enum { EH_ORD_OOB = 0x7FFFFFF0 };
__device__ __forceinline__ void eh_ord_reset(const EhOrd& o, int b, int nblk, int tid, int nthr) {
    const __amdgpu_buffer_rsrc_t rr = eh_ord_rsrc(o.rows, 2 * EH_ORD_ROWS * o.rs);
    const float e = __uint_as_float(EH_ORD_EMPTY);
    const f32x4 ev = {e, e, e, e};
    const int nv = o.soff >> 2;
    for (int r = b; r < o.prev_grid; r += nblk)
        for (int v = tid; v < nv; v += nthr) eh_ord_st16(rr, 4 * (((o.slot ^ 1) * EH_ORD_ROWS + r) * o.rs) + 16 * v, ev);
}
__device__ __forceinline__ void eh_ord_publish(const EhOrd& o, int nth, int tid, int nthr, const float* row, float* flag, unsigned long long* st) {
#ifdef EH_STAMPS
    unsigned long long ts[10];
#endif
    EH_ORD_TICK(ts, 0);
    const unsigned gi = blockIdx.x % EH_ORD_GROUPS, gsz = (gridDim.x - gi + EH_ORD_GROUPS - 1) / EH_ORD_GROUPS;
    const __amdgpu_buffer_rsrc_t rr = eh_ord_rsrc(o.rows, 2 * EH_ORD_ROWS * o.rs);
    const int nv = (nth + 3) >> 2;
#ifdef EH_AB_ORD_PARENT
    asm volatile("s_waitcnt vmcnt(0)" ::: "memory");
#endif
    __syncthreads();
    if (__builtin_amdgcn_readfirstlane(tid >> 6) == 0) {
        const int rb = 4 * ((o.slot * EH_ORD_ROWS + (int)blockIdx.x) * o.rs);
        for (int v = tid; v <= nv; v += 64) {
            const int w = v < nv ? 4 * v : o.soff;
            eh_ord_st16(rr, rb + 4 * w, *(const f32x4*)&row[w]);
        }
        EH_ORD_TICK(ts, 1);
        if (tid == 0) {
            unsigned* const gc = o.cnt + 32 * gi;
            const bool last = __hip_atomic_fetch_add(gc, 1u, __ATOMIC_RELAXED, __HIP_MEMORY_SCOPE_AGENT) == gsz - 1;
            if (last) __hip_atomic_store(gc, 0u, __ATOMIC_RELAXED, __HIP_MEMORY_SCOPE_AGENT);
            flag[0] = last ? 1.0f : 0.0f;
        }
    }
    __syncthreads();
    EH_ORD_TICK(ts, 2);
    if (flag[0] == 0.0f) return;
    constexpr int NK = EH_ORD_ROWS / EH_ORD_GROUPS;
    const int kown = blockIdx.x / EH_ORD_GROUPS;
    const int rb = 4 * ((o.slot * EH_ORD_ROWS + (int)gi) * o.rs), rk = 4 * EH_ORD_GROUPS * o.rs;
    const __amdgpu_buffer_rsrc_t gr = eh_ord_rsrc(o.grows, 2 * EH_ORD_GROUPS * o.rs);
    const int gb = 4 * ((o.slot * EH_ORD_GROUPS + (int)gi) * o.rs);
    for (int v = tid; v < nv; v += nthr) {
        f32x4 r[NK];
#pragma unroll
        for (int k = 0; k < NK; ++k) r[k] = eh_ord_ld16(rr, ((unsigned)k < gsz && k != kown) ? rb + k * rk + 16 * v : (int)EH_ORD_OOB);
        const f32x4 own = *(const f32x4*)&row[4 * v];
        auto fold = [&]() {
            f32x4 s = {0.0f, 0.0f, 0.0f, 0.0f};
#pragma unroll
            for (int k = 0; k < NK; ++k) s += k == kown ? own : r[k];
            return s;
        };
        f32x4 s = fold();
        bool nan = false;
#pragma unroll
        for (int j = 0; j < 4; ++j) nan = nan || (4 * v + j < nth && s[j] != s[j]);
        if (nan) {
            auto empty = [&](int k) {
                bool e = false;
#pragma unroll
                for (int j = 0; j < 4; ++j) e = e || (4 * v + j < nth && __float_as_uint(r[k][j]) == EH_ORD_EMPTY);
                return e;
            };
            bool in = true;
#pragma unroll
            for (int k = 0; k < NK; ++k) in = in && !empty(k);
            if (!in) {
                const unsigned long long t0 = wall_clock64();
                while (true) {
                    __builtin_amdgcn_s_sleep(1);
                    in = true;
#pragma unroll
                    for (int k = 0; k < NK; ++k)
                        if (empty(k)) {
                            r[k] = eh_ord_ld16(rr, rb + k * rk + 16 * v);
                            in = in && !empty(k);
                        }
                    if (in) break;
                    if (wall_clock64() - t0 > EH_ORD_DEADLINE_TICKS) { __hip_atomic_store(o.err, 1u, __ATOMIC_RELAXED, __HIP_MEMORY_SCOPE_SYSTEM); break; }
                }
                s = fold();
            }
        }
        eh_ord_st16(gr, gb + 16 * v, s);
    }
#ifdef EH_STAMPS
    EH_ORD_TICK(ts, 3);
    asm volatile("s_waitcnt vmcnt(0)" ::: "memory");
    EH_ORD_TICK(ts, 4);
    if (st && tid == 0) {
#pragma unroll
        for (int k = 0; k < 10; ++k) st[EH_ORD_ST_TAIL + 10 * gi + k] = ts[k];
    }
#else
    (void)st;
#endif
}

struct EhFused {
    float* gacc;
    float* pset;
    const int* imap;
    float* loss_slot;
    int gslot;
    int cur;
    int sc_sel;
    int pending;
    EhOpt opt;
    float agg_a;
};

struct EhStepArgs {
    const float* recs;
    int C;
    const int* idx;
    long long first, count;
    const float* image;
    float* slab;
    int n_acc;
    const float* inv_n;
    float* yhat;
    const int* rmap;
    float* pout;
    long long yld;
    float shift[EH_MAX_TARG];
    unsigned long long* stamps;
    EhFused fz;
    const float* bn_part;
    int bn_nblk;
    const float* bn_c;
    const float* bn_n;
    int bn_update;
    float* bn_run;
    float* image_out;
    const EhP2P* p2p;
    unsigned p2p_seq;
    EhP2P p2pv;
    const unsigned* prog;
    const unsigned* lprog;
    int ms_nsteps, ms_batch;
    int ms_keep;
    int ms_direct;
    long long ms_end;
    float* ms_loss;
    long long pf_first, pf_count;
    EhOrd ord;
};
enum { EH_LPROG_WORDS = 24 + EH_MAX_PROG };
static_assert(sizeof(long long) == sizeof(unsigned long long), "seed and step of the dropout kernels ride in pf_first / pf_count");
__host__ __device__ inline unsigned long long eh_drop_seed(const EhStepArgs& a) { return (unsigned long long)a.pf_first; }
__host__ __device__ inline unsigned long long eh_drop_step(const EhStepArgs& a) { return (unsigned long long)a.pf_count; }
__host__ inline void eh_drop_set(EhStepArgs& a, unsigned long long seed, unsigned long long step) { a.pf_first = (long long)seed; a.pf_count = (long long)step; }

#define EH_BN_EPS 1e-5f
#define EH_BN_MOMENTUM 0.1f

__device__ __forceinline__ float eh_sigmoid(float x) { return __builtin_amdgcn_rcpf(1.0f + __expf(-x)); }

__device__ __forceinline__ float eh_tanh(float x) {
    const float x2 = x * x;
    const float n = fmaf(x2, fmaf(x2, fmaf(x2, fmaf(x2, 1.587199e-8f, 2.2332108e-5f), 0.0035974074f), 0.1346604f), 1.0f);
    const float d = fmaf(x2, fmaf(x2, fmaf(x2, fmaf(x2, 8.7767893e-7f, 0.0003453992f), 0.026262015f), 0.4679937f), 1.0f);
#ifdef EH_TEST_SKEW
    const float r = 1.001f * x * (n * __builtin_amdgcn_rcpf(d));
// ... 1723 lines not shown
            if (rd == 0) EH_STAMP(12);
            __syncthreads();
            if (rd == 0) EH_STAMP(9);
            {
                float sumv[NU], sumt = 0.0f;
#pragma unroll
                for (int u = 0; u < NU; ++u) {
                    const int wd = min(tid + u * NTHR, KH * 256 - 1);
                    float sum = 0.0f;
#pragma unroll
                    for (int w = 0; w < NW; ++w) sum += R0[w * G::WAVE_WS + wd];
                    sumv[u] = sum;
                }
                if (rd == NR - 1 && tid < 16) {
#pragma unroll
                    for (int w = 0; w < NW; ++w) sumt += R0[w * G::WAVE_WS + KH * 256 + tid];
                }
#pragma unroll
                for (int u = 0; u < NU; ++u)
                    if (dst[u] >= 0) {
                        if (gsh) { if (a.ms_direct) ((eh_lds_f*)gsh)[dst[u]] = sumv[u]; else atomicAdd(&gsh[dst[u]], sumv[u]); }
                        else put_out(dst[u], sumv[u]);
                    }
                if (dtail >= 0) {
                    if (gsh) { if (a.ms_direct) ((eh_lds_f*)gsh)[dtail] = sumt; else atomicAdd(&gsh[dtail], sumt); }
                    else put_out(dtail, sumt);
                }
            }
        }
        if constexpr (P2PM) { if (px_mode == 0) eh_p2p_publish(&a.p2pv, a.fz.gslot, a.p2p_seq, a.n_acc, tid, NTHR); }
        if constexpr (ORDM) eh_ord_publish(a.ord, net.n_theta, tid, NTHR, wl, px_T + 4, a.stamps);
        EH_STAMP_FINE(15);
        if constexpr (!P2PM) { if (a.ms_direct) eh_ms_apply<G>(net, a, gsh, wl, tid, NTHR); }
        EH_STAMP(10);
        return;
    }
    static_assert(!TRAIN || REDV2 || REDV3, "every training shape parks its accumulators the v2 / v3 way");
    EH_STAMP(13);
    __syncthreads();
    EH_STAMP(14);
    float* const RED = smem + G::IMG_FLOATS + wave * a.n_acc;
#pragma unroll
    for (int t = 0; t < EH_MAX_TARG; ++t)
#pragma unroll
        for (int k = 0; k < EH_EVAL_STATS; ++k) {
            const float v = eh_wave_sum(est[t][k]);
            if (t < net.T && lane == 0) RED[t * EH_EVAL_STATS + k] = v;
        }
    EH_STAMP(12);
    __syncthreads();
    EH_STAMP(9);
    {
        const float* const R0 = smem + G::IMG_FLOATS;
        float* const out = a.slab + (long long)blockIdx.x * a.n_acc;
        for (int e = tid; e < a.n_acc; e += NTHR) {
            float s = R0[e];
#pragma unroll
            for (int w = 1; w < NW; ++w) s += R0[w * a.n_acc + e];
            out[e] = s;
        }
    }
    EH_STAMP(10);
}

template <int BYTES>
__device__ __forceinline__ void eh_kernarg_warm() {
#ifndef EH_NO_KERNARG_WARM
    static_assert(BYTES > 192 && BYTES <= 768, "four to twelve lines");
    const auto ka = __builtin_amdgcn_kernarg_segment_ptr();
    unsigned d0, d1, d2, d3, d4 = 0u, d5 = 0u, d6 = 0u, d7 = 0u, d8 = 0u, d9 = 0u, d10 = 0u, d11 = 0u;
    asm volatile("s_load_dword %0, %4, 0x0\n\ts_load_dword %1, %4, 0x40\n\ts_load_dword %2, %4, 0x80\n\ts_load_dword %3, %4, 0xc0"
                 : "=&s"(d0), "=&s"(d1), "=&s"(d2), "=&s"(d3) : "s"(ka));
    if constexpr (BYTES > 0x100) asm volatile("s_load_dword %0, %1, 0x100" : "=&s"(d4) : "s"(ka));
    if constexpr (BYTES > 0x140) asm volatile("s_load_dword %0, %1, 0x140" : "=&s"(d5) : "s"(ka));
    if constexpr (BYTES > 0x180) asm volatile("s_load_dword %0, %1, 0x180" : "=&s"(d6) : "s"(ka));
    if constexpr (BYTES > 0x1c0) asm volatile("s_load_dword %0, %1, 0x1c0" : "=&s"(d7) : "s"(ka));
    if constexpr (BYTES > 0x200) asm volatile("s_load_dword %0, %1, 0x200" : "=&s"(d8) : "s"(ka));
    if constexpr (BYTES > 0x240) asm volatile("s_load_dword %0, %1, 0x240" : "=&s"(d9) : "s"(ka));
    if constexpr (BYTES > 0x280) asm volatile("s_load_dword %0, %1, 0x280" : "=&s"(d10) : "s"(ka));
    if constexpr (BYTES > 0x2c0) asm volatile("s_load_dword %0, %1, 0x2c0" : "=&s"(d11) : "s"(ka));
    asm volatile("s_waitcnt lgkmcnt(0)" ::"s"(d0), "s"(d1), "s"(d2), "s"(d3), "s"(d4), "s"(d5), "s"(d6), "s"(d7), "s"(d8), "s"(d9), "s"(d10), "s"(d11));
#endif
}
#ifdef EH_SPEC_NS
namespace EH_SPEC_NS {
#endif
template <int NBI, int NBH, int NL, int NT, int NW, int ACT, int MODE, int FAST>
__global__ __launch_bounds__(64 * NW, (NW + 3) / 4) void eh_step_kernel(const EhNet net, const EhStepArgs a) {
    eh_kernarg_warm<(int)(sizeof(EhNet) + sizeof(EhStepArgs))>();
    if constexpr (MODE == EH_MODE_TRAIN_MULTI) {
        extern __shared__ __attribute__((aligned(16))) float eh_ms_smem[];
        using G = EhGeom<NBI, NBH, NL, NT, NW>;
        constexpr int NTHR = 64 * NW;
#ifdef EH_SPEC_NET
        constexpr EhNet cnet = {EH_SPEC_NET};
        const int nth = cnet.n_theta, g_off = cnet.g_off;
#else
        const int nth = net.n_theta, g_off = net.g_off;
#endif
        const int np = 6 * nth + (a.fz.opt.tab ? 4 * EH_MAX_OPT_GROUPS : 4), ng = 3 * EH_GSHARDS * a.n_acc + 4;
        float* const l_pset = eh_ms_smem + G::TOTAL_FLOATS;
        float* const l_gacc = l_pset + ((np + 3) & ~3);
        int* const l_imap = reinterpret_cast<int*>(l_gacc + ((ng + 3) & ~3));
        for (int i = threadIdx.x; i < np; i += NTHR) l_pset[i] = a.fz.pset[i];
        for (int i = threadIdx.x; i < ng; i += NTHR) l_gacc[i] = a.fz.gacc[i];
        for (int i = threadIdx.x; i < g_off; i += NTHR) l_imap[i] = a.fz.imap[i];
        __syncthreads();
        EhCarry<(G::IP + 3) / 4> carry;
        carry.valid = false; carry.live = false;
        for (int k = 0; k < a.ms_nsteps; ++k) {
            EhStepArgs b = a;
            b.first = a.first + (long long)k * a.ms_batch;
            const long long left = a.ms_end - b.first;
            b.count = left < (long long)a.ms_batch ? left : (long long)a.ms_batch;
            b.pf_first = b.first + a.ms_batch;
            b.pf_count = k + 1 < a.ms_nsteps ? (left - a.ms_batch < (long long)a.ms_batch ? left - a.ms_batch : (long long)a.ms_batch) : 0;
            if (b.pf_count < 0) b.pf_count = 0;
            b.fz.pset = l_pset; b.fz.gacc = l_gacc; b.fz.imap = l_imap;
            b.fz.gslot = a.fz.gslot;
            b.fz.cur = a.fz.cur;
            b.fz.sc_sel = a.fz.sc_sel;
            b.fz.pending = k ? 0 : a.fz.pending;
            b.fz.loss_slot = a.fz.loss_slot;
            b.ms_loss = a.ms_loss ? a.ms_loss + k : nullptr;
            b.ms_keep = k > 0;
            b.ms_direct = 1;
            eh_step_body<NBI, NBH, NL, NT, NW, ACT, EH_MODE_TRAIN, FAST>(net, b, &carry);
            __syncthreads();
        }
        for (int i = threadIdx.x; i < a.n_acc; i += NTHR) l_gacc[(a.fz.gslot * EH_GSHARDS) * a.n_acc + i] = 0.0f;
        __syncthreads();
        for (int i = threadIdx.x; i < np; i += NTHR) a.fz.pset[i] = l_pset[i];
        for (int i = threadIdx.x; i < ng; i += NTHR) a.fz.gacc[i] = l_gacc[i];
        if (a.image_out)
            for (int i = threadIdx.x; i < G::IMG_FLOATS; i += NTHR) {
                const int q = i - (G::PHI_OFF + EH_IMG_BNM);
                if (q < 0 || q >= 64) a.image_out[i] = eh_ms_smem[i];
            }
    } else {
        eh_step_body<NBI, NBH, NL, NT, NW, ACT, MODE, FAST>(net, a);
    }
}
__host__ __device__ inline long long eh_ms_extra_floats(int n_theta, int n_acc, bool grouped = false) {
    return (long long)((6 * n_theta + (grouped ? 4 * EH_MAX_OPT_GROUPS : 4) + 3) & ~3) + ((3LL * EH_GSHARDS * n_acc + 4 + 3) & ~3LL) + n_theta + 4;
}
#ifdef EH_SPEC_NS
}
using namespace EH_SPEC_NS;
#endif
```

### easyhybrid.jl_amd/csrc/eh_internal.hpp

```cpp
#pragma once
#include <hip/hip_runtime.h>
#include <rccl/rccl.h>

#include <atomic>
#include <cstdarg>
#include <cstdio>
#include <cstdlib>
#include <cstring>
#include <memory>
#include <string>
#include <thread>
#include <vector>

#include "eh_arch.hpp"
#include "eh_jit.hpp"

struct EhImg {
    float* image;
    const int* imap;
    int g_off, phi_off;
    int glob_par[EH_MAX_PARAMS];
    float glo[EH_MAX_PARAMS], ghi[EH_MAX_PARAMS];
    float l2c;
    int b_off;
// ... 59 lines not shown
    float *thb[2] = {nullptr, nullptr}, *mb[2] = {nullptr, nullptr}, *vb[2] = {nullptr, nullptr};
    float* pset = nullptr;
    float* sc = nullptr;
    EhOptTab* opt_tab = nullptr;
    int opt_groups = 1;
    struct EhLbfgs* lb = nullptr;
    int lb_one_max = -1;
    EhChain chain{};
    int chain_gen = 0;
    double* chain_part = nullptr;
    int cur = 0, sc_sel = 0;
    bool fused = false, pending = false, fused_det = false;
    float* gacc = nullptr;
    unsigned* ord = nullptr;
    unsigned* ord_err = nullptr;
    int ord_rs = 0, ord_soff = 0;
    bool pend_ord = false;
    int ord_grid = 0;
    bool p2p_on = false, p2p_alloc = false;
    unsigned long long* p2p_recv = nullptr;
    int p2p_world = 0, p2p_rank = 0;
    unsigned p2p_seq = 0;
    float* p2p_stage = nullptr;
    unsigned* p2p_ctr = nullptr;
    EhP2P* p2p_dev = nullptr;
    EhP2P p2p_host{};
    void* p2p_peer[EH_GSHARDS] = {nullptr};
    eh_handle_s* p2p_group[EH_GSHARDS] = {nullptr};
    bool p2p_local = false;
    long long gstep = 0;
    float* pending_loss = nullptr;
    bool bn_on = false;
    float* bn_part = nullptr;
    float* bn_run = nullptr;
    float* bn_shift = nullptr;
    float* bn_stat = nullptr;
    float* tcount = nullptr;
    float* mombuf = nullptr;
    int mom_stage = 0;
    bool dp_moments = false;
    bool dp_weights = false;
    bool tcount_ready = false;
    bool bn_ext = false;
    bool bn_dp_update = false;
    bool opt_ready = false;
    bool seq = false;
    int seq_I = 0, seq_H = 0, seq_nbi = 0, seq_nbh = 0, seq_act_in = 0, seq_act_hd = 0;
    int seq_off[10] = {0};
    float* seq_ws = nullptr;
    long long seq_ws_floats = 0;
    bool lform = false;
    struct LNet { int nl = 0, c0 = 0, orow = 0, act = 0; int lact[EH_MAX_HIDDEN + 1] = {0}; int in[EH_MAX_HIDDEN + 1] = {0}, out[EH_MAX_HIDDEN + 1] = {0}, woff[EH_MAX_HIDDEN + 1] = {0}, boff[EH_MAX_HIDDEN + 1] = {0}; };
    int l_nnets = 0;
    LNet l_net[EH_MAX_NETS];
    float* l_split = nullptr; size_t l_split_cap = 0;
    unsigned* l_lprog = nullptr; int l_lprog_gen = -1;
    float* l_dk = nullptr; size_t l_dk_cap = 0;
    bool l_job_done = false;
    struct EhLApply* l_apply = nullptr; bool l_applied = false;
    bool l_tail_fn[12] = {false};
    float* l_ws = nullptr;
    long long l_cap = 0;
    unsigned char* wflag = nullptr;
    int slab_rows = 256;
    ncclComm_t comm = nullptr;
    int comm_world = 0, comm_rank = 0;
    struct EhLocalGroup* lgroup = nullptr;
    unsigned roles = 0;
    int agg = 0, n_extra = 0;
    EhOpt opt{};
    EhSplit split[2];
    float *slab = nullptr, *gradbuf = nullptr, *inv_n = nullptr, *loss_hist = nullptr;
    long long loss_cap = 0;
    int* perm = nullptr;
    long long perm_cap = 0;
    bool perm_valid = false;
    int fast_user = 3;
    unsigned* prog = nullptr;
    struct JitEntry { const EhArchInfo* arch; int variant, fast; bool spec, p2p; EhNet net; int loss_gen; float drop[EH_MAX_HIDDEN] = {0}; std::atomic<int> state{0}; EhJitKernel k; std::thread worker; std::string log; bool verified = false; };
    std::vector<std::unique_ptr<JitEntry>> jit;
    bool check_idx = false;
    bool empty_nan = false;
    bool aot_spec = true;
    const struct EhSpecKernel* spec_used = nullptr;
    bool specialize_async = false;
    bool jit_on = true;
    bool jit_failed = false;
    bool specialize = false;
    EhLossProg loss_prog;
    std::string jit_log;
    bool drop_on = false;
    float drop[EH_MAX_HIDDEN] = {0};
    unsigned long long drop_seed = 0, drop_step = 0;
    float* l2val = nullptr;
    float* l2w = nullptr;
    int n_weights = 0;
    struct GraphRec { hipGraphExec_t exec; bool fused; int gslot, cur, sc_sel; bool pend_ord; int ord_grid; bool grouped; int chain_gen; };
    std::vector<GraphRec> graphs;
    bool capturing = false;
    GraphRec cap{};
    int max_blocks = 256;
    bool multi_step = true;
    bool bn_no_self = false;
    int eval_blocks = 0;
    int mech_blocks = 0;
    int mech_tiles = 0;
    float* out_buf = nullptr;
    float* eval_host = nullptr;
    float* eval_host_dev = nullptr;
    size_t eval_host_cap = 0;
    long long out_cap = 0;
    int* idx_buf = nullptr;
    long long idx_cap = 0;
    bool prof = false;
    int prof_stride = 1;
    long long prof_k = 0;
    std::vector<hipEvent_t> ev;
    size_t ev_used = 0;
    unsigned long long* stamps = nullptr;
    std::string err;
};


int fail(eh_handle* h, int code, const char* fmt, ...);
extern std::string g_create_err;
#define HIPCHK(h, expr)                                                                                   \
    do {                                                                                                  \
        hipError_t e_ = (expr);                                                                           \
        if (e_ != hipSuccess) return fail(h, e_ == hipErrorOutOfMemory ? EH_ENOMEM : EH_EHIP, "%s: %s", #expr, hipGetErrorString(e_)); \
    } while (0)

int flush_pending(eh_handle* h);
#define FLUSH(h)                          \
    do {                                  \
        int rc_ = flush_pending(h);       \
        if (rc_) return rc_;              \
    } while (0)

unsigned eh_two_pass_mask(const eh_handle* h);

void eh_comm_release(eh_handle* h);
```

### easyhybrid.jl_amd/csrc/eh_jit.hip

```cpp
#include "eh_jit.hpp"

#include <hip/hiprtc.h>

#include <sys/stat.h>
#include <unistd.h>

#include <cstdio>
#include <cstdlib>
#include <cstring>
#include <vector>

namespace {
#include "eh_sources.inc"

std::string slot_val(unsigned s) {
    char b[32];
    if (s < EH_PROG_SLOT_FORC) snprintf(b, sizeof b, "par[%u]", s);
    else if (s < EH_PROG_SLOT_CONST) snprintf(b, sizeof b, "frc[%u]", s - EH_PROG_SLOT_FORC);
    else if (s < EH_PROG_SLOT_INSTR) snprintf(b, sizeof b, "c%u", s - EH_PROG_SLOT_CONST);
    else snprintf(b, sizeof b, "T.t[%u]", s - EH_PROG_SLOT_INSTR);
    return b;
}
std::string slot_adj(unsigned s) {
    char b[32];
// ... 273 lines not shown
    std::string s = "__device__ __forceinline__ int eh_row_act(int l, int row) {\n";
    char b[96];
    for (int l = 0; l < d.n_hidden; ++l) {
        snprintf(b, sizeof b, "    if (l == %d) return", l);
        s += b;
        if (d.n_nets == 0) {
            snprintf(b, sizeof b, " %d;\n", d.net_activation[l]);
            s += b;
            continue;
        }
        int r0 = 0;
        for (int k = 0; k < d.n_nets; ++k) {
            r0 += d.net_hidden[k][l];
            snprintf(b, sizeof b, " row < %d ? %d :", r0, l < d.net_depth[k] ? d.net_activation[k] : (int)EH_ACT_IDENTITY);
            s += b;
        }
        snprintf(b, sizeof b, " %d;\n", (int)EH_ACT_IDENTITY);
        s += b;
    }
    snprintf(b, sizeof b, "    return %d;\n}\n", (int)EH_ACT_IDENTITY);
    s += b;
    return s;
}

static std::string eh_jit_dropout_source(const float* drop, int n_hidden) {
    std::string t = "__device__ __forceinline__ constexpr unsigned eh_drop_thr(int l) { return", v = "__device__ __forceinline__ constexpr float eh_drop_invp(int l) { return";
    char b[96];
    for (int l = 0; l < n_hidden; ++l) {
        if (!(drop[l] > 0.0f)) continue;
        snprintf(b, sizeof b, " l == %d ? %uu :", l, eh_drop_threshold(drop[l]));
        t += b;
        snprintf(b, sizeof b, " l == %d ? %af :", l, (double)eh_drop_scale(drop[l]));
        v += b;
    }
    return t + " 0u; }\n" + v + " 1.0f; }\n";
}

static thread_local int g_jit_level = 0;
bool eh_jit_build(const eh_model_desc& d, const EhArchInfo* A, int variant, int act, int fast, const EhNet* spec, bool with_p2p,
                  const EhLossProg* loss, EhJitKernel* out, std::string* log, bool allow_slp, const float* drop) {
    const EhVariant& V = A->var[variant];
    const bool prog = d.mech == EH_MECH_PROGRAM;
    const std::string mech = prog ? eh_jit_mech_source(d) : std::string();
    const std::string lsrc = loss ? eh_jit_loss_source(*loss) : std::string();
    const bool rowact = act == EH_ACT_PER_NET;
    const std::string rsrc = rowact ? eh_jit_rowact_source(d) : std::string();
    const std::string dsrc = drop ? eh_jit_dropout_source(drop, d.n_hidden) : std::string();
    std::string src = "typedef signed char int8_t; typedef unsigned char uint8_t; typedef int int32_t; typedef unsigned int uint32_t;\n"
                      "typedef long long int64_t; typedef unsigned long long uint64_t;\n";
    if (const char* dbg = getenv("EH_JIT_DEFINES")) {
        std::string d = dbg;
        size_t at = 0;
        while (at < d.size()) {
            size_t e = d.find(' ', at);
            if (e == std::string::npos) e = d.size();
            if (e > at) {
                std::string tok = d.substr(at, e - at);
                const size_t eq = tok.find('=');
                src += eq == std::string::npos ? "#define " + tok + " 1\n" : "#define " + tok.substr(0, eq) + " " + tok.substr(eq + 1) + "\n";
            }
            at = e + 1;
        }
    }
    if (prog) src += "#define EH_JIT_MECH 1\n";
    if (loss) src += "#define EH_JIT_LOSS 1\n";
    if (rowact) src += "#define EH_JIT_ROWACT 1\n";
    if (drop) src += "#define EH_JIT_DROPOUT 1\n";
    if (spec) {
        char b[512];
        snprintf(b, sizeof b, "#define EH_SPEC_NET %d, %d, %d, %d, %d, %d, %d, %d, %d, %d, %d, %d, %uu, %uu, %uu, %uu, %uu\n", spec->P, spec->K, spec->G, spec->T, spec->F,
                 spec->n_theta, spec->g_off, spec->scale_nn, spec->mech, spec->n_par, spec->loss, spec->n_out, spec->targ_out, spec->par_kind, spec->par_idx, spec->forc_col, spec->loss_t);
        src += b;
    }
    src += V.so ? "#include \"eh_bf16_sample.hpp\"\n" : V.bf16 ? "#include \"eh_wide_bf16.hpp\"\n" : A->wide ? "#include \"eh_wide.hpp\"\n" : "#include \"eh_device.hpp\"\n";
    const char* hnames[9] = {"eh_device.hpp", "eh_wide.hpp", "easyhybrid_hip.h", "eh_wide_bf16.hpp", "eh_bf16_sample.hpp", nullptr, nullptr, nullptr, nullptr};
    const char* hsrc[9] = {eh_src_device, eh_src_wide, eh_src_public, eh_src_widebf, eh_src_bfs, nullptr, nullptr, nullptr, nullptr};
    int nh = 5;
    if (prog) { hnames[nh] = "eh_jit_mech.inc"; hsrc[nh++] = mech.c_str(); }
    if (loss) { hnames[nh] = "eh_jit_loss.inc"; hsrc[nh++] = lsrc.c_str(); }
    if (rowact) { hnames[nh] = "eh_jit_rowact.inc"; hsrc[nh++] = rsrc.c_str(); }
    if (drop) { hnames[nh] = "eh_jit_dropout.inc"; hsrc[nh++] = dsrc.c_str(); }
    hiprtcProgram hp = nullptr;
    if (hiprtcCreateProgram(&hp, src.c_str(), "eh_jit.hip", nh, hsrc, hnames) != HIPRTC_SUCCESS) { *log = "hiprtcCreateProgram failed"; return false; }
    int modes[5], nmode = 0;
    modes[nmode++] = EH_MODE_TRAIN; modes[nmode++] = EH_MODE_EVAL;
    if (with_p2p && !A->wide && !prog) modes[nmode++] = EH_MODE_TRAIN_P2P;
    if (!A->wide && !prog && !loss && !rowact && !drop && spec && spec->T == 1 && !(fast & 4)) { modes[nmode++] = EH_MODE_TRAIN_MULTI; modes[nmode++] = EH_MODE_TRAIN_ORD; }
    char name[5][160];
    for (int i = 0; i < nmode; ++i) {
        const int m = modes[i];
        if (A->wide && V.so && m == EH_MODE_TRAIN) snprintf(name[i], sizeof name[i], "eh_bfs_kernel<%d, %d, %d, %d, %d, %s, %d>", A->nbi, A->nbh, A->nl, V.nw, act, prog ? "true" : "false", V.bf16 == 2 ? 1 : 3);
        else if (A->wide && V.so) snprintf(name[i], sizeof name[i], "eh_widebf_kernel<%d, %d, %d, %d, %d, %d, %d, %s, %d>", A->nbi, A->nbh, A->nl, V.so, V.nw, act, m, prog ? "true" : "false", V.bf16 == 2 ? 1 : 3);
        else if (A->wide && V.bf16) snprintf(name[i], sizeof name[i], "eh_widebf_kernel<%d, %d, %d, %d, %d, %d, %d, %s, %d>", A->nbi, A->nbh, A->nl, V.nt, V.nw, act, m, prog ? "true" : "false", V.bf16 == 2 ? 1 : 3);
        else if (A->wide) snprintf(name[i], sizeof name[i], "eh_wide_kernel<%d, %d, %d, %d, %d, %d, %d, %s>", A->nbi, A->nbh, A->nl, V.nt, V.nw, act, m, prog ? "true" : "false");
        else snprintf(name[i], sizeof name[i], "eh_step_kernel<%d, %d, %d, %d, %d, %d, %d, %d>", A->nbi, A->nbh, A->nl, V.nt, V.nw, act, m,
                      (m == EH_MODE_EVAL) ? (fast & 5) : fast);
        hiprtcAddNameExpression(hp, name[i]);
    }
    const char* const slp_env = getenv("EH_JIT_SLP");
    const bool slp_on = g_jit_level == 0 && allow_slp && (slp_env ? atoi(slp_env) != 0 : (A->nbh == 1 && !A->wide));
    std::vector<std::string> extra;
    if (const char* xo = getenv("EH_JIT_EXTRA_OPTS")) {
        std::string x = xo;
        size_t at = 0;
        while (at < x.size()) {
            size_t e = x.find(' ', at);
            if (e == std::string::npos) e = x.size();
            if (e > at) extra.push_back(x.substr(at, e - at));
            at = e + 1;
        }
    }
    std::vector<const char*> opts = {"--offload-arch=gfx950", g_jit_level >= 2 ? "-O1" : "-O3", slp_on ? "-fslp-vectorize" : "-fno-slp-vectorize", "-std=c++17"};
    for (const std::string& x : extra) opts.push_back(x.c_str());
    std::string cpath;
    {
        const std::string dir = cache_dir();
        if (!dir.empty()) {
            unsigned long long h = 1469598103934665603ull;
            int ver[2] = {0, 0};
            hiprtcVersion(&ver[0], &ver[1]);
            h = fnv(h, ver, sizeof ver);
            h = fnv(h, src.data(), src.size()); h = fnv(h, mech.data(), mech.size()); h = fnv(h, lsrc.data(), lsrc.size()); h = fnv(h, rsrc.data(), rsrc.size());
            h = fnv(h, dsrc.data(), dsrc.size());
            h = fnv(h, eh_src_device, sizeof eh_src_device); h = fnv(h, eh_src_wide, sizeof eh_src_wide); h = fnv(h, eh_src_public, sizeof eh_src_public);
            h = fnv(h, eh_src_widebf, sizeof eh_src_widebf); h = fnv(h, eh_src_bfs, sizeof eh_src_bfs);
            for (int m = 0; m < nmode; ++m) h = fnv(h, name[m], strlen(name[m]));
            for (const char* o : opts) h = fnv(h, o, strlen(o));
            char fn[64];
            snprintf(fn, sizeof fn, "/%016llx.eco", h);
            cpath = dir + fn;
        }
    }
    std::vector<std::string> lowered;
    std::vector<char> code;
    bool from_cache = !cpath.empty() && cache_load(cpath, nmode, &lowered, &code);
    if (getenv("EH_JIT_TRACE")) {
        fprintf(stderr, "eh_jit: %s | slp %d | %s | cache %s%s\n", name[0], (int)slp_on, cpath.c_str(), from_cache ? "hit" : "miss", g_jit_level ? " | retry" : "");
        const size_t at = src.find("#define EH_SPEC_NET");
        if (at != std::string::npos) fprintf(stderr, "eh_jit: %s\n", src.substr(at, src.find('\n', at) - at).c_str());
    }
    if (!from_cache) {
        const char* names[5];
        for (int m = 0; m < nmode; ++m) names[m] = name[m];
        if (!compile_and_cache(hp, opts, names, nmode, cpath, &lowered, &code, log)) {
            hiprtcDestroyProgram(&hp);
            const int next = (g_jit_level == 0 && slp_on) ? 1 : (g_jit_level < 2 ? 2 : 3);
            if (next <= 2) {
                const std::string first = log->substr(0, 240);
                const int saved = g_jit_level;
                g_jit_level = next;
                const bool ok2 = eh_jit_build(d, A, variant, act, fast, spec, with_p2p, loss, out, log, allow_slp, drop);
                g_jit_level = saved;
                if (ok2 && log->empty()) *log = std::string(next == 1 ? "(compiled with -fno-slp-vectorize" : "(compiled at -O1") + " after the first build failed: " + first + ")";
                return ok2;
            }
            return false;
        }
    }
    bool ok = hipModuleLoadData(&out->mod, code.data()) == hipSuccess;
    for (int i = 0; i < nmode && ok; ++i) {
        const int m = modes[i];
        ok = !lowered[i].empty() && hipModuleGetFunction(&out->fn[m], out->mod, lowered[i].c_str()) == hipSuccess;
        if (ok) (void)hipFuncSetAttribute(reinterpret_cast<const void*>(out->fn[m]), hipFuncAttributeMaxDynamicSharedMemorySize,
                                          m == EH_MODE_TRAIN_MULTI ? (int)EH_LDS_LIMIT : (int)V.lds_bytes);
    }
    if (!ok && from_cache) (void)unlink(cpath.c_str());
    (void)hipGetLastError();
    hiprtcDestroyProgram(&hp);
    if (!ok) { *log = "hipModuleLoadData / hipModuleGetFunction failed for the compiled program"; eh_jit_release(out); return false; }
    out->nw = V.nw;
    out->lds_bytes = V.lds_bytes;
    out->lds_eval_bytes = V.lds_eval;
    return true;
}

hipError_t eh_jit_launch(const EhJitKernel* k, int mode, int grid, hipStream_t stream, const EhNet* net, const EhStepArgs* args) {
    void* params[] = {const_cast<EhNet*>(net), const_cast<EhStepArgs*>(args)};
    if (mode < 0 || mode > 4 || !k->fn[mode]) return hipErrorNotSupported;
    if (mode == EH_MODE_TRAIN_MULTI) {
        const size_t lds_ms = k->lds_bytes + sizeof(float) * (size_t)eh_ms_extra_floats(net->n_theta, args->n_acc, args->fz.opt.tab != nullptr);
        if (grid != 1 || lds_ms > EH_LDS_LIMIT) return hipErrorInvalidValue;
        return hipModuleLaunchKernel(k->fn[mode], 1, 1, 1, 64u * (unsigned)k->nw, 1, 1, (unsigned)lds_ms, stream, params, nullptr);
    }
    const size_t lds = (mode == EH_MODE_EVAL && k->lds_eval_bytes) ? k->lds_eval_bytes : k->lds_bytes;
    return hipModuleLaunchKernel(k->fn[mode], (unsigned)grid, 1, 1, 64u * (unsigned)k->nw, 1, 1, (unsigned)lds, stream, params, nullptr);
}

bool eh_jit_build_seq(const eh_model_desc& d, int nbi, int nbh, EhJitKernel* out, std::string* log) {
    if (d.mech != EH_MECH_PROGRAM) { *log = "eh_jit_build_seq: not a recorded closure"; return false; }
    const std::string mech = eh_jit_mech_source(d);
    const std::string src = "typedef signed char int8_t; typedef unsigned char uint8_t; typedef int int32_t; typedef unsigned int uint32_t;\n"
                            "typedef long long int64_t; typedef unsigned long long uint64_t;\n"
                            "#define EH_JIT_MECH 1\n#define EH_SEQ_KERNELS 1\n#include \"eh_seq.hpp\"\n";
    const char* hnames[4] = {"eh_seq.hpp", "eh_device.hpp", "easyhybrid_hip.h", "eh_jit_mech.inc"};
    const char* hsrc[4] = {eh_src_seq, eh_src_device, eh_src_public, mech.c_str()};
    hiprtcProgram hp = nullptr;
    if (hiprtcCreateProgram(&hp, src.c_str(), "eh_jit_seq.hip", 4, hsrc, hnames) != HIPRTC_SUCCESS) { *log = "hiprtcCreateProgram failed"; return false; }
    const int modes[3] = {EH_SEQ_TRAIN, EH_SEQ_EVAL, EH_SEQ_FORWARD};
    char name[3][96];
    for (int i = 0; i < 3; ++i) {
        snprintf(name[i], sizeof name[i], "eh_seq_kernel<%d, %d, %d, %d>", nbi, nbh, modes[i], (int)EH_SEQ_HEAD_PROG);
        hiprtcAddNameExpression(hp, name[i]);
    }
    const std::vector<const char*> opts = {"--offload-arch=gfx950", "-O3", "-fno-slp-vectorize", "-std=c++17"};
    std::string cpath;
    {
        const std::string dir = cache_dir();
        if (!dir.empty()) {
            unsigned long long h = 1469598103934665603ull;
            int ver[2] = {0, 0};
            hiprtcVersion(&ver[0], &ver[1]);
            h = fnv(h, ver, sizeof ver);
            h = fnv(h, src.data(), src.size()); h = fnv(h, mech.data(), mech.size());
            h = fnv(h, eh_src_seq, sizeof eh_src_seq); h = fnv(h, eh_src_device, sizeof eh_src_device); h = fnv(h, eh_src_public, sizeof eh_src_public);
            for (int m = 0; m < 3; ++m) h = fnv(h, name[m], strlen(name[m]));
            for (const char* o : opts) h = fnv(h, o, strlen(o));
            char fn[64];
            snprintf(fn, sizeof fn, "/%016llx.eco", h);
            cpath = dir + fn;
        }
    }
    std::vector<std::string> lowered;
    std::vector<char> code;
    const bool from_cache = !cpath.empty() && cache_load(cpath, 3, &lowered, &code);
    if (getenv("EH_JIT_TRACE")) fprintf(stderr, "eh_jit: %s | %s | cache %s\n", name[0], cpath.c_str(), from_cache ? "hit" : "miss");
    const char* const names[3] = {name[0], name[1], name[2]};
    if (!from_cache && !compile_and_cache(hp, opts, names, 3, cpath, &lowered, &code, log)) { hiprtcDestroyProgram(&hp); return false; }
    bool ok = hipModuleLoadData(&out->mod, code.data()) == hipSuccess;
    for (int i = 0; i < 3 && ok; ++i) ok = !lowered[i].empty() && hipModuleGetFunction(&out->fn[modes[i]], out->mod, lowered[i].c_str()) == hipSuccess;
    if (!ok && from_cache) (void)unlink(cpath.c_str());
    (void)hipGetLastError();
    hiprtcDestroyProgram(&hp);
    if (!ok) { *log = "hipModuleLoadData / hipModuleGetFunction failed for the compiled sequence kernels"; eh_jit_release(out); return false; }
    out->nw = EH_SEQ_NW;
    out->lds_bytes = out->lds_eval_bytes = 0;
    return true;
}

hipError_t eh_jit_launch_seq(const EhJitKernel* k, int mode, int grid, hipStream_t stream, const EhNet* net, const EhSeqArgs* args) {
    void* params[] = {const_cast<EhNet*>(net), const_cast<EhSeqArgs*>(args)};
    if (mode < EH_SEQ_TRAIN || mode > EH_SEQ_FORWARD || !k->fn[mode]) return hipErrorNotSupported;
    return hipModuleLaunchKernel(k->fn[mode], (unsigned)grid, 1, 1, 64u * EH_SEQ_NW, 1, 1, 0, stream, params, nullptr);
}

void eh_jit_release(EhJitKernel* k) {
    if (k->mod) (void)hipModuleUnload(k->mod);
    k->mod = nullptr; k->fn[0] = k->fn[1] = k->fn[2] = k->fn[3] = k->fn[4] = nullptr;
}
```

### easyhybrid.jl_amd/csrc/eh_jit.hpp

```cpp
#pragma once
#include <string>
#include <vector>

#include "eh_arch.hpp"
#include "eh_seq.hpp"

struct EhJitKernel {
    hipModule_t mod = nullptr;
    hipFunction_t fn[5] = {nullptr, nullptr, nullptr, nullptr, nullptr};
    int nw = 0;
    size_t lds_bytes = 0;
    size_t lds_eval_bytes = 0;
};

struct EhLossProg1 {
    std::vector<unsigned> code;
    std::vector<float> consts;
    int out = 0;
};
struct EhLossProg : EhLossProg1 {
    EhLossProg1 per[4];
    int gen = 0;
    const EhLossProg1& of(int t) const { return per[t].code.empty() ? static_cast<const EhLossProg1&>(*this) : per[t]; }
    bool has(int t) const { return !of(t).code.empty(); }
};
std::string eh_jit_loss_source(const EhLossProg& lp);
std::string eh_jit_mech_source(const eh_model_desc& d);
bool eh_jit_build(const eh_model_desc& d, const EhArchInfo* A, int variant, int act, int fast, const EhNet* spec, bool with_p2p,
                  const EhLossProg* loss, EhJitKernel* out, std::string* log, bool allow_slp = true, const float* drop = nullptr);
inline unsigned eh_drop_threshold(float p) { const double t = (double)p * 4294967296.0; return t >= 4294967295.0 ? 4294967295u : (unsigned)t; }
inline float eh_drop_scale(float p) { return 1.0f / (1.0f - p); }
hipError_t eh_jit_launch(const EhJitKernel* k, int mode, int grid, hipStream_t stream, const EhNet* net, const EhStepArgs* args);
void eh_jit_release(EhJitKernel* k);
bool eh_jit_build_seq(const eh_model_desc& d, int nbi, int nbh, EhJitKernel* out, std::string* log);
hipError_t eh_jit_launch_seq(const EhJitKernel* k, int mode, int grid, hipStream_t stream, const EhNet* net, const EhSeqArgs* args);
```

### easyhybrid.jl_amd/csrc/eh_spec.hip

```cpp
#if EH_SPEC_FAMILY == 3
#include "eh_arch.hpp"
#include "eh_bf16_sample.hpp"
#elif EH_SPEC_FAMILY == 2
#include "eh_arch.hpp"
#include "eh_wide_bf16.hpp"
#elif EH_SPEC_FAMILY == 1
#include "eh_arch.hpp"
#include "eh_wide.hpp"
#else
#include "eh_arch.hpp"
#endif

namespace {
constexpr int SH[5] = {EH_SPEC_SHAPE};
constexpr int NBI = SH[0], NBH = SH[1], NL = SH[2], NT = SH[3], NW = SH[4], ACT = EH_SPEC_ACT, FAST = EH_SPEC_FAST;
#ifndef EH_SPEC_NSPLIT
#define EH_SPEC_NSPLIT 3
#endif
#if EH_SPEC_FAMILY == 3
using GeomT = EhBfsGeom<NBI, NBH, NL, NW, EH_SPEC_NSPLIT>;
using GeomE = EhBfGeom<NBI, NBH, NL, EH_SPEC_EVAL_NT, NW, EH_SPEC_NSPLIT>;
struct Geom { static constexpr int TOTAL_FLOATS = GeomT::TOTAL_FLOATS > GeomE::TOTAL_FLOATS ? GeomT::TOTAL_FLOATS : GeomE::TOTAL_FLOATS; };
template <int MODE> struct SpecK;
template <> struct SpecK<EH_MODE_TRAIN> { static constexpr auto fn = &eh_bfs_kernel<NBI, NBH, NL, NW, ACT, false, EH_SPEC_NSPLIT>; };
template <> struct SpecK<EH_MODE_EVAL> { static constexpr auto fn = &eh_widebf_kernel<NBI, NBH, NL, EH_SPEC_EVAL_NT, NW, ACT, EH_MODE_EVAL, false, EH_SPEC_NSPLIT>; };
#define EH_SPEC_KERNEL(MODE) (*SpecK<MODE>::fn)
constexpr bool HASP2P = false;
#elif EH_SPEC_FAMILY == 2
using Geom = EhBfGeom<NBI, NBH, NL, NT, NW, EH_SPEC_NSPLIT>;
#define EH_SPEC_KERNEL(MODE) eh_widebf_kernel<NBI, NBH, NL, NT, NW, ACT, MODE, false, EH_SPEC_NSPLIT>
constexpr bool HASP2P = false;
#elif EH_SPEC_FAMILY == 1
using Geom = EhWideGeom<NBI, NBH, NL, NT, NW>;
#define EH_SPEC_KERNEL(MODE) eh_wide_kernel<NBI, NBH, NL, NT, NW, ACT, MODE, false>
constexpr bool HASP2P = false;
#else
using Geom = EhGeom<NBI, NBH, NL, NT, NW>;
#define EH_SPEC_KERNEL(MODE) eh_step_kernel<NBI, NBH, NL, NT, NW, ACT, MODE, ((MODE) == EH_MODE_EVAL ? (FAST & 5) : FAST)>
constexpr bool HASP2P = (FAST & 4) == 0;
constexpr bool HASMULTI = (FAST & 4) == 0 && EhNet{EH_SPEC_NET}.T == 1;
constexpr bool HASORD = HASMULTI;
#endif
constexpr size_t LDS = sizeof(float) * Geom::TOTAL_FLOATS;
#if EH_SPEC_FAMILY == 0
constexpr size_t LDS_EVAL = sizeof(float) * ((FAST & 1) ? Geom::TOTAL_FLOATS_EVAL_K1 : Geom::TOTAL_FLOATS_EVAL);
#else
constexpr size_t LDS_EVAL = LDS;
#endif
static_assert(LDS <= EH_LDS_LIMIT, "kernel shape does not fit the 160 KiB LDS of a gfx950 CU");

hipError_t prepare() {
    hipError_t e = hipFuncSetAttribute(reinterpret_cast<const void*>(&EH_SPEC_KERNEL(EH_MODE_TRAIN)), hipFuncAttributeMaxDynamicSharedMemorySize, (int)LDS);
    if (e == hipSuccess) e = hipFuncSetAttribute(reinterpret_cast<const void*>(&EH_SPEC_KERNEL(EH_MODE_EVAL)), hipFuncAttributeMaxDynamicSharedMemorySize, (int)LDS);
#if EH_SPEC_FAMILY == 0
    if constexpr (HASP2P) { if (e == hipSuccess) e = hipFuncSetAttribute(reinterpret_cast<const void*>(&EH_SPEC_KERNEL(EH_MODE_TRAIN_P2P)), hipFuncAttributeMaxDynamicSharedMemorySize, (int)LDS); }
    if constexpr (HASORD) { if (e == hipSuccess) e = hipFuncSetAttribute(reinterpret_cast<const void*>(&EH_SPEC_KERNEL(EH_MODE_TRAIN_ORD)), hipFuncAttributeMaxDynamicSharedMemorySize, (int)LDS); }
    if constexpr (HASMULTI) { if (e == hipSuccess) e = hipFuncSetAttribute(reinterpret_cast<const void*>(&EH_SPEC_KERNEL(EH_MODE_TRAIN_MULTI)), hipFuncAttributeMaxDynamicSharedMemorySize, (int)EH_LDS_LIMIT); }
#endif
    return e;
}
hipError_t launch(int mode, int grid, hipStream_t stream, const EhNet* net, const EhStepArgs* args) {
#if EH_SPEC_FAMILY == 3
    if (mode == EH_MODE_TRAIN && args->rmap) return hipErrorNotSupported;
#endif
    if (mode == EH_MODE_TRAIN) hipLaunchKernelGGL((EH_SPEC_KERNEL(EH_MODE_TRAIN)), dim3(grid), dim3(64 * NW), LDS, stream, *net, *args);
    else if (mode == EH_MODE_EVAL) hipLaunchKernelGGL((EH_SPEC_KERNEL(EH_MODE_EVAL)), dim3(grid), dim3(64 * NW), LDS_EVAL, stream, *net, *args);
#if EH_SPEC_FAMILY == 0
    else if (mode == EH_MODE_TRAIN_P2P && HASP2P) hipLaunchKernelGGL((EH_SPEC_KERNEL(EH_MODE_TRAIN_P2P)), dim3(grid), dim3(64 * NW), LDS, stream, *net, *args);
    else if (mode == EH_MODE_TRAIN_ORD && HASORD) hipLaunchKernelGGL((EH_SPEC_KERNEL(EH_MODE_TRAIN_ORD)), dim3(grid), dim3(64 * NW), LDS, stream, *net, *args);
    else if (mode == EH_MODE_TRAIN_MULTI && HASMULTI) {
        const size_t lds_ms = LDS + sizeof(float) * (size_t)eh_ms_extra_floats(net->n_theta, args->n_acc, args->fz.opt.tab != nullptr);
        if (grid != 1 || lds_ms > EH_LDS_LIMIT) return hipErrorInvalidValue;
        hipLaunchKernelGGL((EH_SPEC_KERNEL(EH_MODE_TRAIN_MULTI)), dim3(1), dim3(64 * NW), lds_ms, stream, *net, *args);
    }
#endif
    else return hipErrorNotSupported;
    return hipGetLastError();
}
#define EH_STR_(x) #x
#define EH_STR(x) EH_STR_(x)
const EhSpecKernel spec = {EhNet{EH_SPEC_NET}, EH_SPEC_FAMILY != 0, EH_SPEC_FAMILY >= 2 ? (EH_SPEC_NSPLIT == 3 ? 1 : 2) : 0, NBI, NBH, NL, NT, NW, ACT, FAST, EH_SPEC_FAMILY == 3 ? 1 : 0, LDS,
                           "descriptor " EH_STR(EH_SPEC_ID) " of csrc/Makefile, specialised ahead of time", &prepare, &launch};
}

#define EH_CAT_(a) eh_spec_##a
#define EH_CAT(a) EH_CAT_(a)
extern "C" const EhSpecKernel* EH_CAT(EH_SPEC_ID)(void) { return &spec; }
```

Baseline: 6.224 billion samples/s.

## Add lean train-step kernel variant that folds away unused optional features

Adds a 'lean' template variant of the single-step and ordered train kernels in which batch-norm, inv_n, stamps, multi-step and optimizer-table arguments are forced to null/defaults, so the compiler can drop those branches. Host code decides per handle and per launch whether the configuration qualifies and falls back to the general kernel otherwise. It also rewrites the ordered-reduction spin-wait to poll each peer slot in turn and accumulate directly. The cost is extra compiled kernel variants and more dispatch logic.

New measurement: 6.360 billion samples/s (median of 6 runs). 2.2% higher.

```diff
diff --git a/easyhybrid.jl_amd/csrc/eh_api.hip b/easyhybrid.jl_amd/csrc/eh_api.hip
--- a/easyhybrid.jl_amd/csrc/eh_api.hip
+++ b/easyhybrid.jl_amd/csrc/eh_api.hip
@@ -383,17 +383,56 @@
     return nullptr;
 }
 
+static bool lean_diag_env() { static const bool on = getenv("EH_LEAN_DIAG") != nullptr; return on; }
+static void lean_refresh(eh_handle* h) {
+    static const bool env_off = getenv("EH_NO_LEAN") != nullptr;
+#ifdef EH_STAMPS
+    const bool diag = false;
+#else
+    const bool diag = h->stamps != nullptr && !lean_diag_env();
+#endif
+    h->lean_cfg = h->lean && !env_off && h->arch && !h->arch->wide && !h->lform && !h->seq && h->net.T == 1 && !h->bn_on && !h->drop_on &&
+                  h->net.mech != EH_MECH_PROGRAM && h->net.loss != EH_LOSS_PROGRAM && h->act != EH_ACT_PER_NET && eh_two_pass_mask(h) == 0u &&
+                  h->opt.tab == nullptr && h->opt.rule == EH_OPT_ADAM && !diag;
+}
+static bool lean_wanted(const eh_handle* h, const EhStepArgs* a, bool jit = false) {
+    if (!h->lean_cfg) return false;
+    if (eh_lean_args_ok(*a)) return true;
+    if (!jit || !lean_diag_env() || !a->stamps) return false;
+    EhStepArgs b = *a;
+    b.stamps = nullptr;
+    return eh_lean_args_ok(b);
+}
+static void lean_note(eh_handle* h, bool lean) {
+    const int v = lean ? 1 : 0;
+    if (h->lean_last != v && getenv("EH_JIT_TRACE")) fprintf(stderr, "eh_jit: train step kernel: %s\n", lean ? "lean" : "general");
+    h->lean_last = v;
+}
+
 static hipError_t step_launch(eh_handle* h, int mode, int grid, const EhStepArgs* a) {
     if (mode == EH_MODE_TRAIN_ORD) {
         if (const EhSpecKernel* sk = spec_lookup(h)) {
-            const hipError_t e = sk->launch(mode, grid, h->stream, &h->net, a);
-            if (e == hipSuccess) h->spec_used = sk; else (void)hipGetLastError();
+            bool ln = sk->launch_lean && lean_wanted(h, a);
+            hipError_t e = ln ? sk->launch_lean(mode, grid, h->stream, &h->net, a) : sk->launch(mode, grid, h->stream, &h->net, a);
+            if (ln && e != hipSuccess) {
+                (void)hipGetLastError();
+                ln = false;
+                e = sk->launch(mode, grid, h->stream, &h->net, a);
+            }
+            if (e == hipSuccess) { h->spec_used = sk; lean_note(h, ln); } else (void)hipGetLastError();
             return e;
         }
         if (jit_wanted(h, EH_MODE_TRAIN)) {
             eh_handle_s::JitEntry* je = jit_entry(h);
-            if (je) return (je->verified && je->k.fn[EH_MODE_TRAIN_ORD]) ? eh_jit_launch(&je->k, mode, grid, h->stream, &h->net, a) : hipErrorNotSupported;
-        }
+            if (je) {
+                if (!je->verified || !je->k.fn[EH_MODE_TRAIN_ORD]) return hipErrorNotSupported;
+                const bool ln = je->k.fn_lean[1] && lean_wanted(h, a, true);
+                const hipError_t e = eh_jit_launch(&je->k, mode, grid, h->stream, &h->net, a, ln);
+                if (e == hipSuccess) lean_note(h, ln);
+                return e;
+            }
+        }
+        lean_note(h, false);
         return h->arch->var[h->variant].launch(mode, h->act, KFAST(h), grid, h->stream, &h->net, a);
     }
     if (mode == EH_MODE_TRAIN_MULTI) {
@@ -409,9 +448,16 @@
         }
         return h->arch->var[h->variant].launch(mode, h->act, KFAST(h), grid, h->stream, &h->net, a);
     }
+    const bool train = mode == EH_MODE_TRAIN;
     if (const EhSpecKernel* sk = spec_lookup(h)) {
-        const hipError_t e = sk->launch(mode, grid, h->stream, &h->net, a);
-        if (e == hipSuccess) { h->spec_used = sk; return e; }
+        bool ln = train && sk->launch_lean && lean_wanted(h, a);
+        hipError_t e = ln ? sk->launch_lean(mode, grid, h->stream, &h->net, a) : sk->launch(mode, grid, h->stream, &h->net, a);
+        if (ln && e != hipSuccess) {
+            (void)hipGetLastError();
+            ln = false;
+            e = sk->launch(mode, grid, h->stream, &h->net, a);
+        }
+        if (e == hipSuccess) { h->spec_used = sk; if (train) lean_note(h, ln); return e; }
         (void)hipGetLastError();
     }
     if (jit_wanted(h, mode)) {
@@ -423,8 +469,9 @@
             if (has_lprog || jit_verify(h, je, a)) je->verified = true; else je = nullptr;
         }
         if (je) {
-            const hipError_t e = eh_jit_launch(&je->k, mode, grid, h->stream, &h->net, a);
-            if (e == hipSuccess) return e;
+            const bool ln = train && je->verified && je->k.fn_lean[0] && lean_wanted(h, a, true);
+            const hipError_t e = eh_jit_launch(&je->k, mode, grid, h->stream, &h->net, a, ln);
+            if (e == hipSuccess) { if (train) lean_note(h, ln); return e; }
             (void)hipGetLastError();
             je->state.store(-1); h->jit_failed = true;
             h->jit_log = std::string("launch of the run-time compiled kernel failed: ") + hipGetErrorString(e);
@@ -432,6 +479,7 @@
         if ((h->net.loss == EH_LOSS_PROGRAM || h->drop_on) && mode != EH_MODE_EVAL) return hipErrorNotSupported;
     }
     if (h->act == EH_ACT_PER_NET) return hipErrorNotSupported;
+    if (train) lean_note(h, false);
     return h->arch->var[h->variant].launch(mode, h->act, KFAST(h), grid, h->stream, &h->net, a);
 }
 
@@ -874,6 +922,7 @@
         eh_destroy(h);
         return fail(nullptr, EH_EUNSUPPORTED, "eh_create: per-net activations need the run-time compiled kernel, which failed to build: %.600s", log.c_str());
     }
+    lean_refresh(h);
     *out = h;
     return EH_OK;
 }
@@ -953,6 +1002,7 @@
     lp.consts.assign(consts, consts + n_const);
     lp.out = out_slot;
     h->loss_prog.gen++;
+    lean_refresh(h);
     return EH_OK;
 }
 int32_t eh_set_loss_program(eh_handle* h, const uint32_t* code, int32_t n_instr, const float* consts, int32_t n_const, int32_t out_slot) {
@@ -1018,6 +1068,7 @@
     for (auto& e : h->jit) n += e->state.load(std::memory_order_acquire) > 0 ? 1 : 0;
     std::string msg = h->jit_log;
     if (h->spec_used && h->aot_spec) { n += 1; msg = std::string("ahead-of-time: ") + h->spec_used->what + (msg.empty() ? "" : "; ") + msg; }
+    if (h->lean_last >= 0) msg += std::string(msg.empty() ? "" : "; ") + (h->lean_last ? "train step kernel: lean" : "train step kernel: general");
     *n_compiled = n;
     if (log && log_bytes > 0) {
         const size_t m = std::min((size_t)log_bytes - 1, msg.size());
@@ -1032,8 +1083,14 @@
     return !no_so && h->n_nets == 1 && h->desc.n_nets == 0;
 }
 
+static int32_t set_option(eh_handle* h, const char* name, int64_t value);
 int32_t eh_set_option(eh_handle* h, const char* name, int64_t value) {
     if (!h || !name) return EH_EINVAL;
+    const int32_t rc = set_option(h, name, value);
+    lean_refresh(h);
+    return rc;
+}
+static int32_t set_option(eh_handle* h, const char* name, int64_t value) {
     if (h->seq) {
         if (!strcmp(name, "fused_update")) {
             if (value < 0 || value > 2) return fail(h, EH_EINVAL, "fused_update must be 0, 1 or 2");
@@ -1044,7 +1101,7 @@
             if (value) return fail(h, EH_EUNSUPPORTED, "%s: not built for sequence models (one fp32 kernel family, one launch per step)", name);
             return EH_OK;
         }
-        if (!strcmp(name, "fast_paths") || !strcmp(name, "row_split") || !strcmp(name, "variant") || !strcmp(name, "aot_spec") || !strcmp(name, "bn_in_kernel")) return EH_OK;
+        if (!strcmp(name, "fast_paths") || !strcmp(name, "row_split") || !strcmp(name, "variant") || !strcmp(name, "aot_spec") || !strcmp(name, "bn_in_kernel") || !strcmp(name, "lean")) return EH_OK;
         if (!strcmp(name, "jit")) { h->jit_on = value != 0; return EH_OK; }
         if (!strcmp(name, "training_loss")) {
             if (value < EH_LOSS_MSE || value > EH_LOSS_PROGRAM) return fail(h, EH_EUNSUPPORTED, "training_loss %lld is not implemented on the device", (long long)value);
@@ -1162,6 +1219,10 @@
     }
     if (!strcmp(name, "empty_target_nan")) {
         h->empty_nan = value != 0;
+        return EH_OK;
+    }
+    if (!strcmp(name, "lean")) {
+        h->lean = value != 0;
         return EH_OK;
     }
     if (!strcmp(name, "aot_spec")) {
@@ -2739,6 +2800,7 @@
     HIPCHK(h, hipMemcpy(h->sc, sc, sizeof sc, hipMemcpyHostToDevice));
     h->sc_sel = 0;
     h->opt_ready = true;
+    lean_refresh(h);
     return EH_OK;
 }
 
@@ -2781,6 +2843,7 @@
     HIPCHK(h, hipMemcpy(h->sc, sc, sizeof sc, hipMemcpyHostToDevice));
     h->sc_sel = 0;
     h->opt_ready = true;
+    lean_refresh(h);
     return EH_OK;
 }
 
@@ -3081,6 +3144,7 @@
     for (int l = 0; l < EH_MAX_HIDDEN; ++l) h->drop[l] = (any && l < n_hidden) ? rate[l] : 0.0f;
     h->drop_seed = seed; h->drop_step = step;
     if (any) { h->jit_failed = false; h->jit_log.clear(); }
+    lean_refresh(h);
     return EH_OK;
 }
 
@@ -3549,6 +3613,7 @@
         HIPCHK(h, hipMalloc(&h->stamps, EH_STAMP_WORDS * sizeof(unsigned long long)));
         HIPCHK(h, hipMemset(h->stamps, 0, EH_STAMP_WORDS * sizeof(unsigned long long)));
         memset(out, 0, (size_t)n * sizeof(uint64_t));
+        lean_refresh(h);
         return EH_OK;
     }
     HIPCHK(h, hipStreamSynchronize(h->stream));
diff --git a/easyhybrid.jl_amd/csrc/eh_arch.hpp b/easyhybrid.jl_amd/csrc/eh_arch.hpp
--- a/easyhybrid.jl_amd/csrc/eh_arch.hpp
+++ b/easyhybrid.jl_amd/csrc/eh_arch.hpp
@@ -30,6 +30,7 @@
     const char* what;
     hipError_t (*prepare)(void);
     hipError_t (*launch)(int mode, int grid, hipStream_t stream, const EhNet* net, const EhStepArgs* args);
+    hipError_t (*launch_lean)(int mode, int grid, hipStream_t stream, const EhNet* net, const EhStepArgs* args);
 };
 #define EH_SPEC_LIST(X) X(0) X(1) X(2) X(3) X(4) X(5) X(6)
 #define EH_SPEC_DECL(k) extern "C" const EhSpecKernel* eh_spec_##k(void);
diff --git a/easyhybrid.jl_amd/csrc/eh_device.hpp b/easyhybrid.jl_amd/csrc/eh_device.hpp
--- a/easyhybrid.jl_amd/csrc/eh_device.hpp
+++ b/easyhybrid.jl_amd/csrc/eh_device.hpp
@@ -272,19 +272,28 @@
             for (int k = 0; k < NK; ++k) in = in && !empty(k);
             if (!in) {
                 const unsigned long long t0 = wall_clock64();
-                while (true) {
-                    __builtin_amdgcn_s_sleep(1);
-                    in = true;
-#pragma unroll
-                    for (int k = 0; k < NK; ++k)
-                        if (empty(k)) {
-                            r[k] = eh_ord_ld16(rr, rb + k * rk + 16 * v);
-                            in = in && !empty(k);
+                bool late = false;
+                s = f32x4{0.0f, 0.0f, 0.0f, 0.0f};
+#pragma unroll 1
+                for (int k = 0; k < NK; ++k) {
+                    f32x4 q = own;
+                    if (k != kown) {
+                        const int off = (unsigned)k < gsz ? rb + k * rk + 16 * v : (int)EH_ORD_OOB;
+                        auto empty_q = [&]() {
+                            bool e = false;
+#pragma unroll
+                            for (int j = 0; j < 4; ++j) e = e || (4 * v + j < nth && __float_as_uint(q[j]) == EH_ORD_EMPTY);
+                            return e;
+                        };
+                        q = eh_ord_ld16(rr, off);
+                        while (!late && empty_q()) {
+                            if (wall_clock64() - t0 > EH_ORD_DEADLINE_TICKS) { __hip_atomic_store(o.err, 1u, __ATOMIC_RELAXED, __HIP_MEMORY_SCOPE_SYSTEM); late = true; break; }
+                            __builtin_amdgcn_s_sleep(1);
+                            q = eh_ord_ld16(rr, off);
                         }
-                    if (in) break;
-                    if (wall_clock64() - t0 > EH_ORD_DEADLINE_TICKS) { __hip_atomic_store(o.err, 1u, __ATOMIC_RELAXED, __HIP_MEMORY_SCOPE_SYSTEM); break; }
-                }
-                s = fold();
+                    }
+                    s += q;
+                }
             }
         }
         eh_ord_st16(gr, gb + 16 * v, s);
@@ -2174,6 +2183,27 @@
     asm volatile("s_waitcnt lgkmcnt(0)" ::"s"(d0), "s"(d1), "s"(d2), "s"(d3), "s"(d4), "s"(d5), "s"(d6), "s"(d7), "s"(d8), "s"(d9), "s"(d10), "s"(d11));
 #endif
 }
+enum { EH_FAST_LEAN = 8 };
+__host__ __device__ inline bool eh_lean_args_ok(const EhStepArgs& a) {
+#ifdef EH_STAMPS
+    const bool diag = false;
+#else
+    const bool diag = a.stamps != nullptr;
+#endif
+    return a.bn_part == nullptr && a.bn_nblk != -1 && a.inv_n == nullptr && !diag && a.ms_keep == 0 && a.ms_direct == 0 &&
+           a.fz.opt.tab == nullptr && a.fz.opt.rule == EH_OPT_ADAM;
+}
+__device__ __forceinline__ void eh_lean_fold(EhStepArgs& b) {
+#ifndef EH_AB_NO_LEAN_FOLD
+    b.bn_part = nullptr; b.bn_nblk = 0; b.bn_update = 0; b.bn_n = nullptr; b.bn_c = nullptr; b.bn_run = nullptr;
+    b.inv_n = nullptr;
+#ifndef EH_STAMPS
+    b.stamps = nullptr;
+#endif
+    b.ms_keep = 0; b.ms_direct = 0;
+    b.fz.opt.tab = nullptr; b.fz.opt.rule = EH_OPT_ADAM;
+#endif
+}
 #ifdef EH_SPEC_NS
 namespace EH_SPEC_NS {
 #endif
@@ -2229,6 +2259,11 @@
                 const int q = i - (G::PHI_OFF + EH_IMG_BNM);
                 if (q < 0 || q >= 64) a.image_out[i] = eh_ms_smem[i];
             }
+    } else if constexpr ((FAST & EH_FAST_LEAN) != 0) {
+        static_assert(MODE == EH_MODE_TRAIN || MODE == EH_MODE_TRAIN_ORD, "the lean form exists for the single-step train kernels only");
+        EhStepArgs b = a;
+        eh_lean_fold(b);
+        eh_step_body<NBI, NBH, NL, NT, NW, ACT, MODE, (FAST & ~EH_FAST_LEAN)>(net, b);
     } else {
         eh_step_body<NBI, NBH, NL, NT, NW, ACT, MODE, FAST>(net, a);
     }
diff --git a/easyhybrid.jl_amd/csrc/eh_internal.hpp b/easyhybrid.jl_amd/csrc/eh_internal.hpp
--- a/easyhybrid.jl_amd/csrc/eh_internal.hpp
+++ b/easyhybrid.jl_amd/csrc/eh_internal.hpp
@@ -165,6 +165,9 @@
     bool check_idx = false;
     bool empty_nan = false;
     bool aot_spec = true;
+    bool lean = true;
+    bool lean_cfg = false;
+    int lean_last = -1;
     const struct EhSpecKernel* spec_used = nullptr;
     bool specialize_async = false;
     bool jit_on = true;
diff --git a/easyhybrid.jl_amd/csrc/eh_jit.hip b/easyhybrid.jl_amd/csrc/eh_jit.hip
--- a/easyhybrid.jl_amd/csrc/eh_jit.hip
+++ b/easyhybrid.jl_amd/csrc/eh_jit.hip
@@ -379,11 +379,16 @@
     if (drop) { hnames[nh] = "eh_jit_dropout.inc"; hsrc[nh++] = dsrc.c_str(); }
     hiprtcProgram hp = nullptr;
     if (hiprtcCreateProgram(&hp, src.c_str(), "eh_jit.hip", nh, hsrc, hnames) != HIPRTC_SUCCESS) { *log = "hiprtcCreateProgram failed"; return false; }
-    int modes[5], nmode = 0;
+    int modes[7], nmode = 0;
+    bool lean_k[7] = {false, false, false, false, false, false, false};
     modes[nmode++] = EH_MODE_TRAIN; modes[nmode++] = EH_MODE_EVAL;
     if (with_p2p && !A->wide && !prog) modes[nmode++] = EH_MODE_TRAIN_P2P;
-    if (!A->wide && !prog && !loss && !rowact && !drop && spec && spec->T == 1 && !(fast & 4)) { modes[nmode++] = EH_MODE_TRAIN_MULTI; modes[nmode++] = EH_MODE_TRAIN_ORD; }
-    char name[5][160];
+    if (!A->wide && !prog && !loss && !rowact && !drop && spec && spec->T == 1 && !(fast & 4)) {
+        modes[nmode++] = EH_MODE_TRAIN_MULTI; modes[nmode++] = EH_MODE_TRAIN_ORD;
+        lean_k[nmode] = true; modes[nmode++] = EH_MODE_TRAIN;
+        lean_k[nmode] = true; modes[nmode++] = EH_MODE_TRAIN_ORD;
+    }
+    char name[7][160];
     for (int i = 0; i < nmode; ++i) {
         const int m = modes[i];
         if (A->wide && V.so && m == EH_MODE_TRAIN) snprintf(name[i], sizeof name[i], "eh_bfs_kernel<%d, %d, %d, %d, %d, %s, %d>", A->nbi, A->nbh, A->nl, V.nw, act, prog ? "true" : "false", V.bf16 == 2 ? 1 : 3);
@@ -391,7 +396,7 @@
         else if (A->wide && V.bf16) snprintf(name[i], sizeof name[i], "eh_widebf_kernel<%d, %d, %d, %d, %d, %d, %d, %s, %d>", A->nbi, A->nbh, A->nl, V.nt, V.nw, act, m, prog ? "true" : "false", V.bf16 == 2 ? 1 : 3);
         else if (A->wide) snprintf(name[i], sizeof name[i], "eh_wide_kernel<%d, %d, %d, %d, %d, %d, %d, %s>", A->nbi, A->nbh, A->nl, V.nt, V.nw, act, m, prog ? "true" : "false");
         else snprintf(name[i], sizeof name[i], "eh_step_kernel<%d, %d, %d, %d, %d, %d, %d, %d>", A->nbi, A->nbh, A->nl, V.nt, V.nw, act, m,
-                      (m == EH_MODE_EVAL) ? (fast & 5) : fast);
+                      (m == EH_MODE_EVAL) ? (fast & 5) : lean_k[i] ? (fast | EH_FAST_LEAN) : fast);
         hiprtcAddNameExpression(hp, name[i]);
     }
     const char* const slp_env = getenv("EH_JIT_SLP");
@@ -437,7 +442,7 @@
         if (at != std::string::npos) fprintf(stderr, "eh_jit: %s\n", src.substr(at, src.find('\n', at) - at).c_str());
     }
     if (!from_cache) {
-        const char* names[5];
+        const char* names[7];
         for (int m = 0; m < nmode; ++m) names[m] = name[m];
         if (!compile_and_cache(hp, opts, names, nmode, cpath, &lowered, &code, log)) {
             hiprtcDestroyProgram(&hp);
@@ -457,8 +462,9 @@
     bool ok = hipModuleLoadData(&out->mod, code.data()) == hipSuccess;
     for (int i = 0; i < nmode && ok; ++i) {
         const int m = modes[i];
-        ok = !lowered[i].empty() && hipModuleGetFunction(&out->fn[m], out->mod, lowered[i].c_str()) == hipSuccess;
-        if (ok) (void)hipFuncSetAttribute(reinterpret_cast<const void*>(out->fn[m]), hipFuncAttributeMaxDynamicSharedMemorySize,
+        hipFunction_t& f = lean_k[i] ? out->fn_lean[m == EH_MODE_TRAIN_ORD ? 1 : 0] : out->fn[m];
+        ok = !lowered[i].empty() && hipModuleGetFunction(&f, out->mod, lowered[i].c_str()) == hipSuccess;
+        if (ok) (void)hipFuncSetAttribute(reinterpret_cast<const void*>(f), hipFuncAttributeMaxDynamicSharedMemorySize,
                                           m == EH_MODE_TRAIN_MULTI ? (int)EH_LDS_LIMIT : (int)V.lds_bytes);
     }
     if (!ok && from_cache) (void)unlink(cpath.c_str());
@@ -471,9 +477,14 @@
     return true;
 }
 
-hipError_t eh_jit_launch(const EhJitKernel* k, int mode, int grid, hipStream_t stream, const EhNet* net, const EhStepArgs* args) {
+hipError_t eh_jit_launch(const EhJitKernel* k, int mode, int grid, hipStream_t stream, const EhNet* net, const EhStepArgs* args, bool lean) {
     void* params[] = {const_cast<EhNet*>(net), const_cast<EhStepArgs*>(args)};
     if (mode < 0 || mode > 4 || !k->fn[mode]) return hipErrorNotSupported;
+    if (lean) {
+        const hipFunction_t f = mode == EH_MODE_TRAIN ? k->fn_lean[0] : mode == EH_MODE_TRAIN_ORD ? k->fn_lean[1] : nullptr;
+        if (!f) return hipErrorNotSupported;
+        return hipModuleLaunchKernel(f, (unsigned)grid, 1, 1, 64u * (unsigned)k->nw, 1, 1, (unsigned)k->lds_bytes, stream, params, nullptr);
+    }
     if (mode == EH_MODE_TRAIN_MULTI) {
         const size_t lds_ms = k->lds_bytes + sizeof(float) * (size_t)eh_ms_extra_floats(net->n_theta, args->n_acc, args->fz.opt.tab != nullptr);
         if (grid != 1 || lds_ms > EH_LDS_LIMIT) return hipErrorInvalidValue;
@@ -542,5 +553,5 @@
 
 void eh_jit_release(EhJitKernel* k) {
     if (k->mod) (void)hipModuleUnload(k->mod);
-    k->mod = nullptr; k->fn[0] = k->fn[1] = k->fn[2] = k->fn[3] = k->fn[4] = nullptr;
-}
+    k->mod = nullptr; k->fn[0] = k->fn[1] = k->fn[2] = k->fn[3] = k->fn[4] = nullptr; k->fn_lean[0] = k->fn_lean[1] = nullptr;
+}
diff --git a/easyhybrid.jl_amd/csrc/eh_jit.hpp b/easyhybrid.jl_amd/csrc/eh_jit.hpp
--- a/easyhybrid.jl_amd/csrc/eh_jit.hpp
+++ b/easyhybrid.jl_amd/csrc/eh_jit.hpp
@@ -8,6 +8,7 @@
 struct EhJitKernel {
     hipModule_t mod = nullptr;
     hipFunction_t fn[5] = {nullptr, nullptr, nullptr, nullptr, nullptr};
+    hipFunction_t fn_lean[2] = {nullptr, nullptr};
     int nw = 0;
     size_t lds_bytes = 0;
     size_t lds_eval_bytes = 0;
@@ -30,7 +31,7 @@
                   const EhLossProg* loss, EhJitKernel* out, std::string* log, bool allow_slp = true, const float* drop = nullptr);
 inline unsigned eh_drop_threshold(float p) { const double t = (double)p * 4294967296.0; return t >= 4294967295.0 ? 4294967295u : (unsigned)t; }
 inline float eh_drop_scale(float p) { return 1.0f / (1.0f - p); }
-hipError_t eh_jit_launch(const EhJitKernel* k, int mode, int grid, hipStream_t stream, const EhNet* net, const EhStepArgs* args);
+hipError_t eh_jit_launch(const EhJitKernel* k, int mode, int grid, hipStream_t stream, const EhNet* net, const EhStepArgs* args, bool lean = false);
 void eh_jit_release(EhJitKernel* k);
 bool eh_jit_build_seq(const eh_model_desc& d, int nbi, int nbh, EhJitKernel* out, std::string* log);
 hipError_t eh_jit_launch_seq(const EhJitKernel* k, int mode, int grid, hipStream_t stream, const EhNet* net, const EhSeqArgs* args);
diff --git a/easyhybrid.jl_amd/csrc/eh_spec.hip b/easyhybrid.jl_amd/csrc/eh_spec.hip
--- a/easyhybrid.jl_amd/csrc/eh_spec.hip
+++ b/easyhybrid.jl_amd/csrc/eh_spec.hip
@@ -40,6 +40,10 @@
 constexpr bool HASP2P = (FAST & 4) == 0;
 constexpr bool HASMULTI = (FAST & 4) == 0 && EhNet{EH_SPEC_NET}.T == 1;
 constexpr bool HASORD = HASMULTI;
+#ifdef EH_SPEC_LEAN
+#define EH_SPEC_KERNEL_LEAN(MODE) eh_step_kernel<NBI, NBH, NL, NT, NW, ACT, MODE, (FAST | EH_FAST_LEAN)>
+static_assert(HASORD, "the lean form is built for descriptors that have the ordered step");
+#endif
 #endif
 constexpr size_t LDS = sizeof(float) * Geom::TOTAL_FLOATS;
 #if EH_SPEC_FAMILY == 0
@@ -56,6 +60,10 @@
     if constexpr (HASP2P) { if (e == hipSuccess) e = hipFuncSetAttribute(reinterpret_cast<const void*>(&EH_SPEC_KERNEL(EH_MODE_TRAIN_P2P)), hipFuncAttributeMaxDynamicSharedMemorySize, (int)LDS); }
     if constexpr (HASORD) { if (e == hipSuccess) e = hipFuncSetAttribute(reinterpret_cast<const void*>(&EH_SPEC_KERNEL(EH_MODE_TRAIN_ORD)), hipFuncAttributeMaxDynamicSharedMemorySize, (int)LDS); }
     if constexpr (HASMULTI) { if (e == hipSuccess) e = hipFuncSetAttribute(reinterpret_cast<const void*>(&EH_SPEC_KERNEL(EH_MODE_TRAIN_MULTI)), hipFuncAttributeMaxDynamicSharedMemorySize, (int)EH_LDS_LIMIT); }
+#ifdef EH_SPEC_LEAN
+    if (e == hipSuccess) e = hipFuncSetAttribute(reinterpret_cast<const void*>(&EH_SPEC_KERNEL_LEAN(EH_MODE_TRAIN)), hipFuncAttributeMaxDynamicSharedMemorySize, (int)LDS);
+    if (e == hipSuccess) e = hipFuncSetAttribute(reinterpret_cast<const void*>(&EH_SPEC_KERNEL_LEAN(EH_MODE_TRAIN_ORD)), hipFuncAttributeMaxDynamicSharedMemorySize, (int)LDS);
+#endif
 #endif
     return e;
 }
@@ -77,10 +85,22 @@
     else return hipErrorNotSupported;
     return hipGetLastError();
 }
+#ifdef EH_SPEC_LEAN
+hipError_t launch_lean(int mode, int grid, hipStream_t stream, const EhNet* net, const EhStepArgs* args) {
+    if (!eh_lean_args_ok(*args)) return hipErrorInvalidValue;
+    if (mode == EH_MODE_TRAIN) hipLaunchKernelGGL((EH_SPEC_KERNEL_LEAN(EH_MODE_TRAIN)), dim3(grid), dim3(64 * NW), LDS, stream, *net, *args);
+    else if (mode == EH_MODE_TRAIN_ORD) hipLaunchKernelGGL((EH_SPEC_KERNEL_LEAN(EH_MODE_TRAIN_ORD)), dim3(grid), dim3(64 * NW), LDS, stream, *net, *args);
+    else return hipErrorNotSupported;
+    return hipGetLastError();
+}
+constexpr auto LAUNCH_LEAN = &launch_lean;
+#else
+constexpr hipError_t (*LAUNCH_LEAN)(int, int, hipStream_t, const EhNet*, const EhStepArgs*) = nullptr;
+#endif
 #define EH_STR_(x) #x
 #define EH_STR(x) EH_STR_(x)
 const EhSpecKernel spec = {EhNet{EH_SPEC_NET}, EH_SPEC_FAMILY != 0, EH_SPEC_FAMILY >= 2 ? (EH_SPEC_NSPLIT == 3 ? 1 : 2) : 0, NBI, NBH, NL, NT, NW, ACT, FAST, EH_SPEC_FAMILY == 3 ? 1 : 0, LDS,
-                           "descriptor " EH_STR(EH_SPEC_ID) " of csrc/Makefile, specialised ahead of time", &prepare, &launch};
+                           "descriptor " EH_STR(EH_SPEC_ID) " of csrc/Makefile, specialised ahead of time", &prepare, &launch, LAUNCH_LEAN};
 }
 
 #define EH_CAT_(a) eh_spec_##a
```
